# Meeso1/nmmo

Measured on AMD Instinct MI355X. Metric: agent-steps/sec (whole node), 128-agent envs at 1/2/4/8 MI355X, higher is better.
Workload: dtype int16

## Files before the change

### nmmo_amd/csrc/agent_obs.h

```cpp
#pragma once

#include <utility>

#include "kernels.h"
#include "wire.h"

namespace nmmo {

#ifndef NMMO_AO_WAVES
#define NMMO_AO_WAVES 4
#define NMMO_AO_AGENTS 16
#endif
constexpr int kAoWaves = NMMO_AO_WAVES;
constexpr int kAoAgents = NMMO_AO_AGENTS;
constexpr int kAoRows = kMaxSlots / 64;
constexpr uint32_t kAoEmpty = 0xFFFFFFFFu;
static_assert(kSize <= 256 && kMaxSlots <= 2 * 256 && kMaxSlots % 64 == 0, "packed entity word; two slots per thread (>= 256 threads)");
__host__ __device__ constexpr int ao_stride(int S) { return ((S + 1) >> 1 | 1) << 1; }
__host__ __device__ constexpr size_t ao_columns_lds(int S) {
  return ((size_t)NMMO_N_ENTITY_COLS * ao_stride(S) * 2 + 15) & ~(size_t)15;
}
constexpr size_t kAoPkBytes = (size_t)(kMaxSlots + 64) * 4;
__host__ __device__ constexpr size_t ao_entity_lds(int S) { return ao_columns_lds(S) + kAoPkBytes; }
__host__ __device__ inline uint32_t ao_pack(int slot, int row, int col, bool immune, bool danger, bool player) {
  return (uint32_t)(row & 255) | (uint32_t)(slot & 255) << 8 | (uint32_t)(col & 255) << 16 | (uint32_t)(slot >> 8) << 24 |
         (immune ? 1u << 25 : 0u) | (danger ? 1u << 26 : 0u) | (player ? 1u << 27 : 0u);
}
__device__ __forceinline__ int ao_slot(uint32_t w) { return (int)(((w >> 8) & 255u) | ((w >> 16) & 256u)); }
__device__ __forceinline__ int ao_row(uint32_t w) { return (int)(w & 255u); }
__device__ __forceinline__ int ao_col(uint32_t w) { return (int)((w >> 16) & 255u); }
__device__ __forceinline__ bool ao_immune(uint32_t w) { return (w >> 25) & 1u; }
__device__ __forceinline__ bool ao_danger(uint32_t w) { return (w >> 26) & 1u; }
__device__ __forceinline__ bool ao_player(uint32_t w) { return (w >> 27) & 1u; }
typedef unsigned short ao_u16x2 __attribute__((ext_vector_type(2)));
__device__ __forceinline__ bool ao_in_window(uint32_t w, uint32_t rc) {
  ao_u16x2 d = __builtin_bit_cast(ao_u16x2, w & 0x00FF00FFu) - __builtin_bit_cast(ao_u16x2, rc) +
               (ao_u16x2){(unsigned short)kVision, (unsigned short)kVision};
  return (d.x > d.y ? d.x : d.y) <= 2 * kVision;
}
static_assert(kMaxSlots <= 512 && kSize <= 255, "packed entity word");

__device__ __forceinline__ int ao_lane() {
  int l = (int)(threadIdx.x & 63u);
  asm volatile("" : "+v"(l));
  return l;
}

__device__ __forceinline__ uint64_t low_bits(int n) { return n >= 64 ? ~0ull : n <= 0 ? 0ull : (1ull << n) - 1ull; }
template <int L>
__device__ __forceinline__ int writelane(int v, int x) {
  static_assert(L >= 0 && L < 64, "lane");
  int sv = __builtin_amdgcn_readfirstlane(v);
  asm volatile("" : "+s"(sv));
  asm volatile("v_writelane_b32 %0, %1, %2" : "+v"(x) : "s"(sv), "n"(L));
  return x;
}
template <int kLane0, int kIdx0, int... D>
__device__ __forceinline__ int writelanes_(const uint32_t* img, int x, std::integer_sequence<int, D...>) {
  ((x = writelane<kLane0 + D>((int)img[kIdx0 + D], x)), ...);
  return x;
}
template <int kLane0, int kIdx0, int kN>
__device__ __forceinline__ int writelanes(const uint32_t* img, int x) {
  return writelanes_<kLane0, kIdx0>(img, x, std::make_integer_sequence<int, kN>{});
}

template <int kOff, int kN, int kW>
__device__ __forceinline__ void put_field(uint32_t (&img)[kW], uint64_t lo, uint64_t hi) {
  static_assert((kOff + kN + 31) / 32 <= kW, "image size");
#pragma unroll
  for (int d = kOff / 32; d <= (kOff + kN - 1) / 32; d++) {
    const int st = 32 * d - kOff;
    uint32_t x;
    if (st < 0) x = (uint32_t)(lo << (-st));
    else if (st == 0) x = (uint32_t)lo;
    else if (st < 64) x = (uint32_t)((lo >> st) | (hi << (64 - st)));
    else x = (uint32_t)(hi >> (st - 64));
    img[d] |= x;
  }
}

constexpr int kAoStageIt = (NMMO_N_ENTITY_COLS * (kMaxSlots / 8) + 255) / 256;
struct AoStage {
  uint4 x[kAoStageIt];
  int al[2], ds[2];
  int nm, mv;
};
template <bool kAligned = true>
__device__ __forceinline__ void ao_stage_load(const ObsParams& p, int e, AoStage& r) {
  const int S = p.S, tid = threadIdx.x;
  const int16_t* E = p.ent + (size_t)e * NMMO_NF * S;
  const int w4 = S / 8;
  const int nw = NMMO_N_ENTITY_COLS * w4;
  r.nm = p.mcount[e];
  r.mv = p.mlist[(size_t)e * NMMO_MARKET_ROWS + min(tid, NMMO_MARKET_ROWS - 1)];
  if constexpr (kAligned) {
#pragma unroll
    for (int k = 0; k < kAoStageIt; k++) {
      const int i = tid + (int)blockDim.x * k;
      const int f = i / w4, j = i - f * w4;
      r.x[k] = i < nw ? reinterpret_cast<const uint4*>(E + (size_t)f * S)[j] : make_uint4(0u, 0u, 0u, 0u);
    }
  }
#pragma unroll
  for (int u = 0; u < 2; u++) {
    const int s = min(tid + (int)blockDim.x * u, S - 1);
    r.al[u] = E[F_ALIVE * S + s];
    r.ds[u] = E[F_DS_ROW * S + s];
  }
}
template <bool kAligned = true>
__device__ __forceinline__ void ao_stage_store(const ObsParams& p, int e, int16_t* T, uint32_t* pk, const AoStage& r) {
  const int S = p.S, P = p.P, Sp = ao_stride(S), tid = threadIdx.x;
  const int16_t* E = p.ent + (size_t)e * NMMO_NF * S;
  const int w4 = S / 8;
  const int nw = NMMO_N_ENTITY_COLS * w4;
  constexpr int kIt = kAoStageIt;
  const int(&al)[2] = r.al;
  const int(&ds)[2] = r.ds;
  if constexpr (kAligned) {
#pragma unroll
    for (int k = 0; k < kIt; k++) {
      const int i = tid + (int)blockDim.x * k;
      if (i < nw) {
        const int f = i / w4, j = i - f * w4;
        uint32_t* d = reinterpret_cast<uint32_t*>(T + f * Sp) + 4 * j;
        d[0] = r.x[k].x;
        d[1] = r.x[k].y;
        d[2] = r.x[k].z;
        d[3] = r.x[k].w;
      }
    }
    for (int i = tid + (int)blockDim.x * kIt; i < nw; i += blockDim.x) {
      const int f = i / w4, j = i - f * w4;
      const uint4 y = reinterpret_cast<const uint4*>(E + (size_t)f * S)[j];
      uint32_t* d = reinterpret_cast<uint32_t*>(T + f * Sp) + 4 * j;
      d[0] = y.x;
      d[1] = y.y;
      d[2] = y.z;
      d[3] = y.w;
    }
  } else {
    for (int i = tid; i < NMMO_N_ENTITY_COLS * S; i += blockDim.x) {
      const int f = i / S;
      T[f * Sp + i - f * S] = E[i];
    }
  }
  for (int k = tid; k < kMaxSlots + 64; k += blockDim.x) pk[k] = kAoEmpty;
  __syncthreads();
#pragma unroll
  for (int u = 0; u < 2; u++) {
    const int s = tid + (int)blockDim.x * u;
    if (s < S && al[u] && (unsigned)(ds[u] - 1) < (unsigned)S) {
      const bool player = s < P;
      const bool immune = player && T[F_TIME_ALIVE * Sp + s] < p.spawn_immunity;
      const bool danger = T[F_NPC_TYPE * Sp + s] > 1;
      pk[ds[u] - 1] = ao_pack(s, T[F_ROW * Sp + s], T[F_COL * Sp + s], immune, danger, player);
    }
  }
  __syncthreads();
}
__device__ __forceinline__ uint2 ao_listing_load(const ObsParams& p, int e, const AoStage& r) {
  const int own = min((r.mv >> 16) & 255, p.P - 1), slot = min((r.mv >> 24) & 15, kInv - 1);
  return p.items[((size_t)e * p.P + own) * kInv + slot];
}

constexpr int kAoWinRowBytes = 20;
constexpr int kAoWinAgentBytes = 15 * kAoWinRowBytes;
__host__ __device__ constexpr size_t ao_win_lds(int agents = kAoAgents) {
  return (size_t)agents * kAoWinAgentBytes + (size_t)agents * kInv * 8;
}
__device__ __forceinline__ int ao_clamp_pos(int x) { return min(max(x, kVision), kSize - 1 - kVision); }
struct AoNoop {
  __device__ void operator()() const {}
};
template <int kAgents = kAoAgents, int kRowDw = kAoWinRowBytes / 4, typename F = AoNoop, typename B = AoNoop>
__device__ inline void ao_stage_windows(const ObsParams& p, int e, int g, const int16_t* T, int Sp, uint32_t* ws, uint2* is,
                                        F before_barrier = F(), B before_writes = B()) {
  static_assert(kRowDw == 4 || kRowDw == 5, "window row: 5 aligned dwords, or 4 realigned");
  const int tid = threadIdx.x, P = p.P;
  const int la = tid / 15, row = tid - 15 * la, a = g * kAgents + la;
  const bool win = tid < kAgents * 15 && a < P;
  uint32_t d[5] = {0u, 0u, 0u, 0u, 0u};
  if (win) {
    const int r = ao_clamp_pos(T[F_ROW * Sp + a]), c = ao_clamp_pos(T[F_COL * Sp + a]);
    const int base = (r - kVision + row) * kSize + c - kVision;
    const uint32_t* src = reinterpret_cast<const uint32_t*>(p.mat + (size_t)e * kTiles) + (base >> 2);
#pragma unroll
    for (int k = 0; k < 5; k++) d[k] = src[k];
    if constexpr (kRowDw == 4) {
#pragma unroll
      for (int k = 0; k < 4; k++) d[k] = __builtin_amdgcn_alignbyte(d[k + 1], d[k], (uint32_t)(c - kVision) & 3u);
    }
  }
  uint2 iw = make_uint2(0u, 0u);
  const bool itm = tid < kAgents * kInv && g * kAgents + tid / kInv < P;
  if (itm) iw = p.items[((size_t)e * P + g * kAgents) * kInv + tid];
  before_writes();
  if (win) {
#pragma unroll
    for (int k = 0; k < kRowDw; k++) ws[tid * kRowDw + k] = d[k];
  }
  if (tid < kAgents * kInv) is[tid] = iw;
  before_barrier();
  __syncthreads();
}
template <int kRowBytes = kAoWinRowBytes>
__device__ __forceinline__ void ao_win_offsets(int (&wo)[2]) {
  wo[0] = wo[1] = 0;
#pragma unroll
  for (int i = 0; i < 4; i++) {
    const int t = lane_id() + 64 * i;
    const int o = t < 225 ? (t / 15) * kRowBytes + t % 15 : 0;
    wo[i >> 1] |= o << (16 * (i & 1));
  }
}
__device__ __forceinline__ int ao_win_off(const int (&wo)[2], int i) { return (wo[i >> 1] >> (16 * (i & 1))) & 0xFFFF; }

__device__ __forceinline__ int ao_compact(const uint32_t (&pr)[kAoRows], int S, int r, int c, uint32_t* visw) {
  int nvis = 0;
  const uint32_t rc = (uint32_t)r | (uint32_t)c << 16;
#pragma unroll
  for (int i = 0; i < kAoRows; i++) {
    if (64 * i >= S) break;
    const uint32_t x = pr[i];
    const bool in = ao_in_window(x, rc);
    const uint64_t b = __ballot(in);
    const int pos = nvis + __popcll(b & lanes_below());
    if (in && pos < kNObs) visw[pos] = x;
    nvis += __popcll(b);
  }
  return nvis;
}

__device__ __forceinline__ void ao_window_offsets(int (&mo)[2]) {
  mo[0] = mo[1] = 0;
#pragma unroll
  for (int i = 0; i < 4; i++) {
    const int t = lane_id() + 64 * i;
    const int o = t < 225 ? (t / 15 - kVision) * kSize + t % 15 - kVision : 0;
    mo[i >> 1] |= (o & 0xFFFF) << (16 * (i & 1));
  }
}
__device__ __forceinline__ int ao_window_off(const int (&mo)[2], int i) {
  return (int)(int16_t)(uint16_t)((uint32_t)mo[i >> 1] >> (16 * (i & 1)));
}

static_assert(F_ALCHEMY_LEVEL == F_MELEE_LEVEL + 14 && F_FISHING_LEVEL == F_MELEE_LEVEL + 6 &&
                  F_HERBALISM_LEVEL == F_MELEE_LEVEL + 8, "skill level fields");
__host__ __device__ constexpr uint64_t ao_req_lut() {
  uint64_t m = 0;
  for (int t = 0; t < 16; t++) {
    const int k = (t >= T_SPEAR && t <= T_WAND) ? t - T_SPEAR : (t >= T_WHETSTONE && t <= T_RUNES) ? t - T_WHETSTONE
                  : (t >= T_ROD && t <= T_CHISEL) ? 3 + t - T_ROD : 8;
    m |= (uint64_t)k << (4 * t);
  }
  return m;
}
static_assert(T_RATION == 16 && T_POTION == 17, "requirement table: ration -> fishing, potion -> herbalism");
__device__ __forceinline__ uint64_t ao_usable_ballot(const int16_t* T, int Sp, int ti, uint2 it, bool have) {
  const int lane = ao_lane();
  int lv = 0;
  if (lane < 8) {
    lv = T[(F_MELEE_LEVEL + 2 * lane) * Sp + ti];
  } else if (lane == 8) {
    lv = max((int)T[F_MELEE_LEVEL * Sp + ti], max((int)T[F_RANGE_LEVEL * Sp + ti], (int)T[F_MAGE_LEVEL * Sp + ti]));
  }
  const int type = it_type(it);
  const int k = type < 16 ? (int)((ao_req_lut() >> (4 * type)) & 15u) : type == T_RATION ? 3 : type == T_POTION ? 4 : 8;
  const int req = __shfl(lv, k);
  const bool eq = type >= T_HAT && type <= T_RUNES && it_equipped(it);
  return __ballot(have && !it_price(it) && (eq || it_level(it) <= req));
}

struct AoSections {
  uint64_t s0, s1[2], s3, s4, s5[2], s6[2], s7[2], s8, s9, s10[2], s11;
};
struct AoAgent {
  int a, ti, r, c, gold, aid, nv, ninv, prev_price;
  uint32_t mv;
};
template <bool kWrap>
__device__ __forceinline__ AoSections ao_sections(const ObsParams& p, const int16_t* T, int Sp, const uint32_t* visw,
                                                 const AoAgent& g, uint2 it) {
  const bool combat = (p.systems & NMMO_SYS_COMBAT) != 0;
  const bool item = (p.systems & NMMO_SYS_ITEM) != 0;
  const bool exch = item && (p.systems & NMMO_SYS_EXCHANGE) != 0;
  const bool no_give = kWrap && (p.wflags & kWrapObsNoGive);
  const bool no_danger = kWrap && (p.wflags & kWrapObsNoDangerous);
  const int lane = ao_lane();
  AoSections x;
  x.s1[0] = x.s1[1] = x.s5[0] = x.s5[1] = x.s7[0] = x.s7[1] = 0ull;
#pragma unroll
  for (int h = 0; h < 2; h++) {
    if (64 * h >= g.nv) break;
    const int k = 64 * h + lane;
    bool tgt = false, st = false;
    if (k < g.nv) {
      const uint32_t w = visw[k];
      const int q = ao_slot(w);
      tgt = combat && q != g.a && linf(g.r, g.c, ao_row(w), ao_col(w)) <= 3 && !ao_immune(w) &&
            !(no_danger && ao_danger(w));
      st = ao_player(w) && q != g.a && ao_row(w) == g.r && ao_col(w) == g.c;
    }
    x.s1[h] = __ballot(tgt);
    const uint64_t sb = __ballot(st);
    if (item && !no_give) x.s5[h] = sb;
    if (exch && !no_give) x.s7[h] = sb;
  }
  x.s1[1] |= 1ull << (kNObs - 64);
  x.s5[1] |= 1ull << (kNObs - 64);
  x.s7[1] |= 1ull << (kNObs - 64);
  const bool have = lane < g.ninv;
  const bool fr = have && !it_equipped(it) && !it_price(it);
  const uint64_t bfr = __ballot(fr);
  x.s3 = (item ? bfr : 0ull) | 1ull << kInv;
  x.s4 = (item && !no_give ? bfr : 0ull) | 1ull << kInv;
  x.s9 = (exch ? __ballot(have && !it_equipped(it)) : 0ull) | 1ull << kInv;
  x.s11 = (item ? ao_usable_ballot(T, Sp, g.ti, it, have) : 0ull) | 1ull << kInv;
  x.s0 = combat ? low_bits(kSecN[0]) : 0ull;
  x.s6[0] = x.s6[1] = x.s10[0] = x.s10[1] = 0ull;
  if (exch) {
    const int ng = no_give ? min(g.gold, 1) : min(g.gold, kSecN[6]);
    x.s6[0] = low_bits(ng);
    x.s6[1] = low_bits(ng - 64);
    x.s10[0] = low_bits(kSecN[10]);
    x.s10[1] = low_bits(kSecN[10] - 64);
    if constexpr (kWrap) {
      const int pp = g.prev_price;
      if ((p.wflags & kWrapObsPrice) && pp >= 0 && pp < kSecN[10]) {
        const uint64_t clr = ~(1ull << (pp & 63));
        if (pp < 64) x.s10[0] &= clr;
        else x.s10[1] &= clr;
      }
    }
  }
  x.s8 = g.mv;
  return x;
}

template <bool kFlat, int kW>
__device__ __forceinline__ void ao_image(const AoSections& x, uint32_t (&img)[kW]) {
#pragma unroll
  for (int d = 0; d < kW; d++) img[d] = 0u;
#define AO_PUT(k, lo, hi) put_field<kFlat ? sec_flat(k) : sec_wire(k), kSecN[k], kW>(img, lo, hi)
  AO_PUT(0, x.s0, 0ull);
  AO_PUT(1, x.s1[0], x.s1[1]);
  AO_PUT(3, x.s3, 0ull);
  AO_PUT(4, x.s4, 0ull);
  AO_PUT(5, x.s5[0], x.s5[1]);
  AO_PUT(6, x.s6[0], x.s6[1]);
  AO_PUT(7, x.s7[0], x.s7[1]);
  AO_PUT(8, x.s8, 0ull);
  AO_PUT(9, x.s9, 0ull);
  AO_PUT(10, x.s10[0], x.s10[1]);
  AO_PUT(11, x.s11, 0ull);
#undef AO_PUT
}

}
```

### nmmo_amd/csrc/capi.hip

```cpp
#include <math.h>
#include <stdlib.h>
#include <string.h>

#include <algorithm>
#include <map>
#include <mutex>
#include <vector>

#include "host_api.h"
#include "kernels.h"
#include "wire.h"

using namespace nmmo;

#define HIP_TRY(expr)                                                                    \
  do {                                                                                   \
    hipError_t _e = (expr);                                                              \
    if (_e != hipSuccess) return fail(NMMO_E_HIP, "%s: %s", #expr, hipGetErrorString(_e)); \
  } while (0)

struct NmmoHandle {
  NmmoConfig cfg;
  NmmoLayout layout;
  DevState st;
  int device;
  int32_t* d_env = nullptr;
  int16_t* d_ent = nullptr;
  int16_t* d_ring = nullptr;
  uint8_t* d_mat = nullptr;
  uint32_t* d_dep = nullptr;
  int32_t* d_foreign = nullptr;
  uint8_t* d_bank = nullptr;
  float* d_task = nullptr;
  uint64_t* d_seeds = nullptr;
  uint2* d_items = nullptr;
  int16_t* d_iring = nullptr;
  int32_t* d_mlist = nullptr;
  int32_t* d_mcount = nullptr;
  int32_t* d_events = nullptr;
  NmmoTask* d_tasks = nullptr;
  int32_t* d_assign = nullptr;
  NmmoTaskState* d_tstate = nullptr;
  uint16_t* d_wcount = nullptr;
  int32_t* d_wmcount = nullptr;
  uint16_t* d_wrank = nullptr;
  uint32_t* d_wpk = nullptr;
  uint64_t* d_zrow = nullptr;
  uint64_t* d_zext = nullptr;
  bool zskip = true;
  bool wire_fuse = true;
  const void* zbuf = nullptr;
  uint64_t ztag = 0;
  unsigned long long* d_rows_out = nullptr;
  uint8_t* d_recs = nullptr;
  int32_t* d_recs_fault = nullptr;
  const void* last_native = nullptr;
  bool native_fresh = false;
  bool wrap_on = false;
  NmmoWrapperConfig wc{};
  NmmoWrapState* d_ws = nullptr;
  uint32_t* d_uniq = nullptr;
  int32_t* d_wenv = nullptr;
  uint64_t* d_task_cum = nullptr;
  unsigned long long* d_wdrop = nullptr;
  NmmoAgentInfo* d_info = nullptr;
  bool timing = false;
  int t_count = 0;
  std::vector<hipEvent_t> ev;
};
static constexpr int kTimingCap = 8192;

static float half_to_float(uint16_t h) {
  uint32_t s = (uint32_t)(h >> 15) << 31, e = (h >> 10) & 31, m = h & 1023, bits;
  if (e == 0) {
    if (m == 0) {
      bits = s;
    } else {
      int sh = 0;
      while (!(m & 1024)) { m <<= 1; sh++; }
      m &= 1023;
      bits = s | ((uint32_t)(127 - 15 - sh + 1) << 23) | (m << 13);
    }
  } else if (e == 31) {
    bits = s | 0x7F800000u | (m << 13);
  } else {
    bits = s | ((e + 112) << 23) | (m << 13);
  }
  float f;
  memcpy(&f, &bits, 4);
  return f;
}

extern "C" {

int32_t nmmo_abi_version(void) { return NMMO_ABI_VERSION; }
const char* nmmo_build_info(void) {
  return NMMO_BUILD_INFO
#ifdef NMMO_STAMPS
         " stamps=1"
#endif
      ;
}
const char* nmmo_last_error(void) { return g_err.c_str(); }

void nmmo_default_config(NmmoConfig* c) {
  memset(c, 0, sizeof(*c));
  c->abi_version = NMMO_ABI_VERSION;
  c->player_n = 128;
  c->npc_n = 256;
  c->horizon = 1024;
  c->map_n = 256;
  c->spawn_immunity = 20;
  c->early_stop_agent_num = 0;
  c->resilient_u32 = 858993459u;
  c->systems = NMMO_SYS_ALL;
  c->obs_layout = NMMO_OBS_FLAT;
  c->task_embed_dim = 2048;
  c->task_num_tick = 1024;
  c->event_cap = 4096;
  c->map_seed = 0;
  c->env_index_base = 0;
}

int nmmo_layout(const NmmoConfig* cfg, NmmoLayout* L) {
  if (!cfg || !L) return fail(NMMO_E_INVALID, "null argument");
  memset(L, 0, sizeof(*L));
  L->act_heads = NMMO_N_ACTION_HEADS;
  int* offs[NMMO_N_ACTION_HEADS] = {
      &L->off_mask_attack_style, &L->off_mask_attack_target, &L->off_mask_buy,
      &L->off_mask_destroy, &L->off_mask_give_item, &L->off_mask_give_target,
      &L->off_mask_givegold_price, &L->off_mask_givegold_target, &L->off_mask_move,
      &L->off_mask_sell_item, &L->off_mask_sell_price, &L->off_mask_use};
  for (int h = 0; h < NMMO_N_ACTION_HEADS; h++) {
    L->act_dims[h] = kSecN[h];
    *offs[h] = sec_flat(h);
  }
  L->off_agent_id = kFlatId;
  L->off_current_tick = kFlatTick;
  L->off_entity = kFlatEntity;
  L->off_inventory = kFlatInv;
  L->off_market = kFlatMarket;
  L->off_task = kFlatTask;
  L->off_tile = flat_tile(cfg->task_embed_dim);
  L->obs_elems = flat_elems(cfg->task_embed_dim);
  L->entity_rows = kNObs; L->entity_cols = NMMO_N_ENTITY_COLS;
  L->inventory_rows = kInv; L->item_cols = kItemCols; L->market_rows = NMMO_MARKET_ROWS;
  L->tile_rows = kWinTiles; L->tile_cols = kTileCols;
  const int npc = (cfg->systems & NMMO_SYS_NPC) ? cfg->npc_n : 0;
  L->slots = cfg->player_n + npc;
  L->nf = NMMO_NF;
  L->ne = NMMO_NE;
  L->state_bytes_per_env = (size_t)NMMO_NE * 4 + (size_t)NMMO_NF * L->slots * 2 +
                           (size_t)L->slots * 2 + NMMO_MAP_TILES +
                           (size_t)cfg->player_n * NMMO_INV_SLOTS * 8 +
                           (size_t)NMMO_INV_SLOTS * cfg->player_n * 2 + (size_t)cfg->player_n * 4 +
                           (size_t)cfg->player_n * sizeof(NmmoTaskState);
  return NMMO_OK;
}

int32_t nmmo_n_envs(const NmmoHandle* h) { return h ? h->st.n_envs : 0; }

void nmmo_destroy(NmmoHandle* h) {
  if (!h) return;
  (void)hipSetDevice(h->device);
  for (hipEvent_t e : h->ev) (void)hipEventDestroy(e);
  void* bufs[] = {h->d_env,  h->d_ent,   h->d_ring,  h->d_mat,   h->d_dep,   h->d_bank,
                  h->d_task, h->d_seeds, h->d_items, h->d_iring, h->d_mlist, h->d_mcount,
                  h->d_events, h->d_tasks, h->d_assign, h->d_tstate, h->d_ws, h->d_uniq, h->d_wenv, h->d_wdrop, h->d_task_cum,
                  h->d_wcount, h->d_wmcount, h->d_wrank, h->d_wpk, h->d_foreign, h->d_zrow, h->d_zext};
  for (void* b : bufs)
    if (b) (void)hipFree(b);
  delete h;
}

int nmmo_create(const NmmoConfig* cfg, int32_t n_envs, uint64_t seed, int32_t device,
                const uint16_t* task_embedding, NmmoHandle** out) {
  if (!cfg || !out) return fail(NMMO_E_INVALID, "null argument");
  *out = nullptr;
  if (cfg->abi_version != NMMO_ABI_VERSION)
    return fail(NMMO_E_INVALID, "abi_version %d != %d", cfg->abi_version, NMMO_ABI_VERSION);
  if (n_envs <= 0) return fail(NMMO_E_INVALID, "n_envs must be > 0");
  if (cfg->player_n <= 0 || cfg->player_n > 128) return fail(NMMO_E_INVALID, "player_n in 1..128");
  if (cfg->npc_n < 0 || cfg->npc_n > 256) return fail(NMMO_E_INVALID, "npc_n in 0..256");
  if (cfg->map_n <= 0) return fail(NMMO_E_INVALID, "map_n must be > 0");
  if (cfg->horizon <= 0 || cfg->task_num_tick <= 0) return fail(NMMO_E_INVALID, "horizon/task_num_tick");
  if (cfg->task_embed_dim < 0 || cfg->task_embed_dim > 65536) return fail(NMMO_E_INVALID, "task_embed_dim");
  if (cfg->event_cap < 0 || cfg->event_cap > (1 << 24)) return fail(NMMO_E_INVALID, "event_cap in 0..2^24");
  if (cfg->obs_layout != NMMO_OBS_NONE && cfg->obs_layout != NMMO_OBS_FLAT && cfg->obs_layout != NMMO_OBS_NATIVE &&
      cfg->obs_layout != NMMO_OBS_WIRE)
    return fail(NMMO_E_INVALID, "obs_layout %d", cfg->obs_layout);
  NmmoHandle* h = new NmmoHandle();
  h->cfg = *cfg;
  h->device = device;
  nmmo_layout(cfg, &h->layout);
  const int P = cfg->player_n, N = (cfg->systems & NMMO_SYS_NPC) ? cfg->npc_n : 0, S = P + N;
  auto cleanup_fail = [&](int code) { nmmo_destroy(h); return code; };
  if (hipSetDevice(device) != hipSuccess) return cleanup_fail(fail(NMMO_E_HIP, "hipSetDevice(%d)", device));
  const size_t n = (size_t)n_envs;
#define ALLOC(ptr, bytes)                                                               \
  if (hipMalloc((void**)&(ptr), (bytes)) != hipSuccess)                                  \
    return cleanup_fail(fail(NMMO_E_NOMEM, "hipMalloc %zu bytes for %s", (size_t)(bytes), #ptr)); \
  if (hipMemset((ptr), 0, (bytes)) != hipSuccess) return cleanup_fail(fail(NMMO_E_HIP, "hipMemset"));
  ALLOC(h->d_env, n * NMMO_NE * 4);
  ALLOC(h->d_ent, n * NMMO_NF * S * 2);
  ALLOC(h->d_ring, n * S * 2);
  ALLOC(h->d_mat, n * NMMO_MAP_TILES);
  ALLOC(h->d_dep, n * kBitmapWords * 4);
  ALLOC(h->d_foreign, 8);
  ALLOC(h->d_bank, (size_t)cfg->map_n * NMMO_MAP_TILES);
  ALLOC(h->d_task, (size_t)(cfg->task_embed_dim > 0 ? cfg->task_embed_dim : 1) * 4);
  ALLOC(h->d_seeds, n * 8);
  ALLOC(h->d_items, n * P * NMMO_INV_SLOTS * 8);
  ALLOC(h->d_iring, n * NMMO_INV_SLOTS * P * 2);
  ALLOC(h->d_mlist, n * NMMO_MARKET_ROWS * 4);
  ALLOC(h->d_mcount, n * 4);
  if (cfg->event_cap > 0) ALLOC(h->d_events, n * (size_t)cfg->event_cap * NMMO_EVENT_COLS * 4);
  ALLOC(h->d_tasks, sizeof(NmmoTask));
  ALLOC(h->d_assign, n * P * 4);
  ALLOC(h->d_tstate, n * P * sizeof(NmmoTaskState));
  if (cfg->obs_layout == NMMO_OBS_NATIVE) {
    ALLOC(h->d_wcount, n * P * 2);
    ALLOC(h->d_wmcount, n * 4);
  }
  if (cfg->obs_layout == NMMO_OBS_FLAT || cfg->obs_layout == NMMO_OBS_NATIVE) {
    ALLOC(h->d_zrow, n * P * 16);
  }
  if (cfg->obs_layout == NMMO_OBS_FLAT) {
    ALLOC(h->d_zext, n * P * kZext * 8);
  }
  {
    const char* rz = getenv("NMMO_OBS_REZERO");
    h->zskip = !(rz && rz[0] == '1');
    const char* wf = getenv("NMMO_WIRE_FUSE");
    h->wire_fuse = !(wf && wf[0] == '0');
  }
  if (cfg->obs_layout == NMMO_OBS_WIRE) {
    ALLOC(h->d_wrank, n * (size_t)kMaxSlots * 2);
    ALLOC(h->d_wpk, n * (size_t)kMaxSlots * 4);
  }
#undef ALLOC
  if (init_kernels() != hipSuccess) return cleanup_fail(fail(NMMO_E_HIP, "kernel attributes"));
  if (task_embedding && cfg->task_embed_dim > 0) {
    std::vector<float> t(cfg->task_embed_dim);
    for (int k = 0; k < cfg->task_embed_dim; k++) t[k] = half_to_float(task_embedding[k]);
    if (hipMemcpy(h->d_task, t.data(), t.size() * 4, hipMemcpyHostToDevice) != hipSuccess)
      return cleanup_fail(fail(NMMO_E_HIP, "task upload"));
  }
  h->st = DevState{h->d_env,   h->d_ent,   h->d_ring,  h->d_mat,    h->d_dep, h->d_bank,
                   h->d_items, h->d_iring, h->d_mlist, h->d_mcount, h->d_events,
                   h->d_tasks, h->d_assign, nullptr, h->d_tstate, 1,            0,           0, 0, n_envs, P,
                   N,          S,          seed,       nullptr,     *cfg,      h->d_foreign,
                   h->d_foreign + 1, nullptr, 0};
  {
    NmmoTask t;
    memset(&t, 0, sizeof(t));
    t.term[0].pred = PRED_TICK_GE;
    t.term[0].a = cfg->task_num_tick;
    if (hipMemcpy(h->d_tasks, &t, sizeof(t), hipMemcpyHostToDevice) != hipSuccess)
      return cleanup_fail(fail(NMMO_E_HIP, "task table upload"));
  }
  if (launch_mapgen(cfg->map_seed, cfg->map_n, h->d_bank, nullptr) != hipSuccess ||
      hipDeviceSynchronize() != hipSuccess)
    return cleanup_fail(fail(NMMO_E_HIP, "map generation failed: %s", hipGetErrorString(hipGetLastError())));
  *out = h;
  return NMMO_OK;
}

static ObsParams obs_params(NmmoHandle* h, void* obs) {
  ObsParams p;
  const bool native = h->cfg.obs_layout == NMMO_OBS_NATIVE, wire = h->cfg.obs_layout == NMMO_OBS_WIRE;
  p.env = h->d_env; p.ent = h->d_ent; p.mat = h->d_mat; p.task = h->d_task;
  p.obs = native || wire ? nullptr : (float*)obs;
  p.nat = native ? (uint8_t*)obs : nullptr;
  p.wire = wire ? (uint8_t*)obs : nullptr;
  p.items = h->d_items; p.mlist = h->d_mlist; p.mcount = h->d_mcount; p.assign = h->d_assign;
  p.n_envs = h->st.n_envs; p.P = h->st.P; p.S = h->st.S;
  p.task_dim = h->cfg.task_embed_dim; p.systems = h->cfg.systems;
  p.spawn_immunity = h->cfg.spawn_immunity;
  p.row_map = nullptr;
  p.env_list = nullptr;
  p.n_list = 0;
  p.wcount = native ? h->d_wcount : nullptr;
  p.wmcount = native ? h->d_wmcount : nullptr;
  p.wrank = wire ? h->d_wrank : nullptr;
  p.wpk = wire ? h->d_wpk : nullptr;
  p.fault = h->d_foreign + 1;
  p.zrow = h->d_zrow;
  p.zst = h->d_zrow ? h->d_zrow + (size_t)h->st.n_envs * h->st.P : nullptr;
  p.zext = h->d_zext;
  p.ztag = h->d_zrow && h->zskip && obs && obs == h->zbuf ? h->ztag : 0;
  p.rows_out = h->d_rows_out;
  p.counted = 0;
  p.recs = nullptr;
  p.fault_dst = nullptr;
  p.rew = nullptr;
  p.term = p.trunc = p.mask = nullptr;
  p.ws = h->wrap_on ? h->d_ws : nullptr;
  p.wflags = 0;
  if (h->wrap_on) {
    if (h->wc.kind == NMMO_WRAP_START_KIT) p.wflags |= kWrapObsPrice;
    if (h->wc.disable_give) p.wflags |= kWrapObsNoGive;
    if (h->wc.donot_attack_dangerous_npc) p.wflags |= kWrapObsNoDangerous;
  }
  return p;
}

static WrapParams wrap_params(NmmoHandle* h, const int32_t* actions, float* rew, const uint8_t* term,
                              const uint8_t* trunc, const uint8_t* mask) {
  WrapParams p;
  p.env = h->d_env; p.ent = h->d_ent; p.items = h->d_items; p.events = h->d_events;
  p.tstate = h->d_tstate; p.actions = actions; p.rew = rew; p.term = term; p.trunc = trunc;
  p.mask = mask; p.ws = h->d_ws; p.uniq = h->d_uniq; p.wenv = h->d_wenv; p.wdrop = h->d_wdrop; p.info = h->d_info;
  p.wc = h->wc; p.n_envs = h->st.n_envs; p.P = h->st.P; p.S = h->st.S; p.evcap = h->cfg.event_cap;
  p.items_on = (h->cfg.systems & NMMO_SYS_ITEM) != 0;
  p.env_list = nullptr;
  p.n_list = 0;
  return p;
}

int nmmo_reset(NmmoHandle* h, const uint64_t* env_seeds, void* obs, uint8_t* mask, void* stream) {
  if (!h) return fail(NMMO_E_INVALID, "null handle");
  hipStream_t s = (hipStream_t)stream;
  HIP_TRY(hipSetDevice(h->device));
  if (env_seeds) {
    HIP_TRY(hipMemcpyAsync(h->d_seeds, env_seeds, (size_t)h->st.n_envs * 8, hipMemcpyHostToDevice, s));
    HIP_TRY(hipStreamSynchronize(s));
  }
  HIP_TRY(launch_tick(h->st, nullptr, env_seeds ? h->d_seeds : nullptr, nullptr, nullptr, nullptr,
                      mask, 1, s));
  HIP_TRY(hipMemsetAsync(h->d_foreign, 0, 4, s));
  if (h->wrap_on) HIP_TRY(launch_wrap(wrap_params(h, nullptr, nullptr, nullptr, nullptr, nullptr), 0, s));
  const bool do_obs = obs && h->cfg.obs_layout != NMMO_OBS_NONE;
  if (do_obs) HIP_TRY(launch_obs(obs_params(h, obs), s));
  if (do_obs) h->last_native = obs;
  h->native_fresh = do_obs;
  return NMMO_OK;
}

__global__ void end_episodes_kernel(int32_t* env, const uint8_t* m, int n) {
  const int e = blockIdx.x * blockDim.x + threadIdx.x;
  if (e < n && m[e]) env[(size_t)e * NMMO_NE + E_DONE] = 1;
}

int nmmo_end_episodes(NmmoHandle* h, const uint8_t* dev_env_mask, void* stream) {
  if (!h || !dev_env_mask) return fail(NMMO_E_INVALID, "null argument");
  const int n = h->st.n_envs;
  HIP_TRY(hipSetDevice(h->device));
  hipLaunchKernelGGL(end_episodes_kernel, dim3((n + 255) / 256), dim3(256), 0, (hipStream_t)stream, h->d_env,
                     dev_env_mask, n);
  HIP_TRY(hipGetLastError());
  return NMMO_OK;
}

static int step_impl(NmmoHandle* h, const int32_t* env_ids, int32_t n_ids, const int32_t* actions, void* obs,
                     float* rew, uint8_t* term, uint8_t* trunc, uint8_t* mask, void* stream) {
  if (!h) return fail(NMMO_E_INVALID, "null handle");
  if (!actions || !rew || !term || !trunc || !mask)
    return fail(NMMO_E_INVALID, "actions/rew/term/trunc/mask must be device pointers");
  HIP_TRY(hipSetDevice(h->device));
  hipStream_t s = (hipStream_t)stream;
  const bool rec = h->timing && h->t_count < kTimingCap;
  hipEvent_t* ev = rec ? &h->ev[(size_t)h->t_count * 4] : nullptr;
  DevState st = h->st;
  st.env_list = env_ids;
  st.n_list = n_ids;
  const bool do_obs = obs && h->cfg.obs_layout != NMMO_OBS_NONE;
  if (do_obs && h->cfg.obs_layout == NMMO_OBS_WIRE && !env_ids && !h->wrap_on && h->wire_fuse &&
      st.cfg.systems == NMMO_SYS_ALL && st.S == 384 && st.P == 128) {
    st.wf.wire = (uint8_t*)obs;
    st.wf.wrank = h->d_wrank;
    st.wf.wpk = h->d_wpk;
    st.wf.n_envs = st.n_envs;
    st.wf.spawn_immunity = h->cfg.spawn_immunity;
  }
  if (rec) HIP_TRY(hipEventRecord(ev[0], s));
  HIP_TRY(launch_tick(st, actions, nullptr, rew, term, trunc, mask, 0, s));
  if (rec) HIP_TRY(hipEventRecord(ev[1], s));
  if (h->wrap_on) {
    WrapParams wp = wrap_params(h, actions, rew, term, trunc, mask);
    wp.env_list = env_ids;
    wp.n_list = n_ids;
    HIP_TRY(launch_wrap(wp, 0, s));
  }
  if (rec) HIP_TRY(hipEventRecord(ev[2], s));
  if (do_obs) {
    ObsParams op = obs_params(h, obs);
    op.env_list = env_ids;
    op.n_list = n_ids;
    op.counted = st.wf.wire != nullptr;
    if (op.wire && h->d_recs) {
      op.recs = h->d_recs;
      op.fault_dst = h->d_recs_fault;
      op.rew = rew;
      op.term = term;
      op.trunc = trunc;
      op.mask = mask;
    }
    HIP_TRY(launch_obs(op, s));
  }
  if (do_obs) h->last_native = obs;
  h->native_fresh = do_obs && !env_ids;
  if (rec) {
    HIP_TRY(hipEventRecord(ev[3], s));
    h->t_count++;
  }
  return NMMO_OK;
}

int nmmo_step(NmmoHandle* h, const int32_t* actions, void* obs, float* rew, uint8_t* term,
              uint8_t* trunc, uint8_t* mask, void* stream) {
  return step_impl(h, nullptr, 0, actions, obs, rew, term, trunc, mask, stream);
}

int nmmo_step_envs(NmmoHandle* h, const int32_t* env_ids, int32_t n_ids, const int32_t* actions, void* obs,
                   float* rew, uint8_t* term, uint8_t* trunc, uint8_t* mask, void* stream) {
  if (!h || !env_ids) return fail(NMMO_E_INVALID, "null handle / env_ids");
  if (n_ids < 0 || n_ids > h->st.n_envs) return fail(NMMO_E_INVALID, "n_ids %d not in 0..%d", n_ids, h->st.n_envs);
  if (h->cfg.obs_layout == NMMO_OBS_WIRE && obs)
    return fail(NMMO_E_INVALID, "nmmo_step_envs: the wire layout packs every env of the handle (use nmmo_step)");
  return step_impl(h, env_ids, n_ids, actions, obs, rew, term, trunc, mask, stream);
}

__global__ void fault_into_kernel(const int32_t* word, int32_t* dst) {
  const int32_t w = *word;
  if (w) atomicCAS(dst, 0, w);
}

int nmmo_fault_into(NmmoHandle* h, int32_t* dev_dst, void* stream) {
  if (!h || !dev_dst) return fail(NMMO_E_INVALID, "null argument");
  HIP_TRY(hipSetDevice(h->device));
  hipLaunchKernelGGL(fault_into_kernel, dim3(1), dim3(1), 0, (hipStream_t)stream, h->d_foreign + 1, dev_dst);
  HIP_TRY(hipGetLastError());
  return NMMO_OK;
}

int nmmo_inject_fault(NmmoHandle* h, int32_t fault) {
  if (!h) return fail(NMMO_E_INVALID, "null handle");
  HIP_TRY(hipSetDevice(h->device));
  HIP_TRY(hipDeviceSynchronize());
  HIP_TRY(hipMemcpy(h->d_foreign + 1, &fault, 4, hipMemcpyHostToDevice));
  return NMMO_OK;
}

int nmmo_observe(NmmoHandle* h, void* obs, void* stream) {
  if (!h || !obs) return fail(NMMO_E_INVALID, "null argument");
  if (h->cfg.obs_layout == NMMO_OBS_NONE) return fail(NMMO_E_INVALID, "handle built with NMMO_OBS_NONE");
  HIP_TRY(hipSetDevice(h->device));
  HIP_TRY(launch_obs(obs_params(h, obs), (hipStream_t)stream));
  h->last_native = obs;
  h->native_fresh = true;
  return NMMO_OK;
}

int nmmo_expand_obs(NmmoHandle* h, const void* native, float* flat, int32_t n_envs, void* stream) {
  if (!h || !native || !flat) return fail(NMMO_E_INVALID, "null argument");
  if (n_envs <= 0) return fail(NMMO_E_INVALID, "n_envs must be > 0");
  ObsParams p = obs_params(h, nullptr);
  p.nat = (uint8_t*)native;
  p.obs = flat;
  p.n_envs = n_envs;
  HIP_TRY(launch_expand(p, (hipStream_t)stream));
  return NMMO_OK;
}

namespace {
struct VmmAlloc {
  size_t bytes;
  std::vector<hipMemGenericAllocationHandle_t> chunks;
};
std::mutex g_vmm_mu;
std::map<void*, VmmAlloc> g_vmm;
constexpr size_t kVmmChunk = (size_t)64 << 20;
}

int nmmo_dev_alloc(int32_t device, uint64_t bytes, void** out) {
  if (!out || bytes == 0) return fail(NMMO_E_INVALID, "null out / zero bytes");
  *out = nullptr;
  HIP_TRY(hipSetDevice(device));
  int vmm = 0;
  HIP_TRY(hipDeviceGetAttribute(&vmm, hipDeviceAttributeVirtualMemoryManagementSupported, device));
  if (!vmm) return fail(NMMO_E_INVALID, "device %d has no virtual memory management (hipMemCreate / hipMemMap)", device);
  hipMemAllocationProp prop = {};
  prop.type = hipMemAllocationTypePinned;
  prop.location.type = hipMemLocationTypeDevice;
  prop.location.id = device;
  size_t gran = 0;
  HIP_TRY(hipMemGetAllocationGranularity(&gran, &prop, hipMemAllocationGranularityMinimum));
  const size_t chunk = gran > kVmmChunk ? gran : (kVmmChunk / gran) * gran;
  const size_t total = (bytes + chunk - 1) / chunk * chunk;
  void* va = nullptr;
  HIP_TRY(hipMemAddressReserve(&va, total, chunk, nullptr, 0));
  VmmAlloc a{total, {}};
  size_t mapped = 0;
  auto undo = [&]() {
    for (size_t i = 0; i < mapped; i++) (void)hipMemUnmap((char*)va + i * chunk, chunk);
    for (auto c : a.chunks) (void)hipMemRelease(c);
    (void)hipMemAddressFree(va, total);
  };
  for (size_t off = 0; off < total; off += chunk) {
    hipMemGenericAllocationHandle_t hdl;
    if (hipMemCreate(&hdl, chunk, &prop, 0) != hipSuccess) {
      undo();
      return fail(NMMO_E_NOMEM, "hipMemCreate of a %zu-byte chunk (%zu of %zu mapped)", chunk, off, total);
    }
    a.chunks.push_back(hdl);
    if (hipMemMap((char*)va + off, chunk, 0, hdl, 0) != hipSuccess) {
      undo();
      return fail(NMMO_E_HIP, "hipMemMap at offset %zu", off);
    }
    mapped++;
  }
  hipMemAccessDesc acc = {};
  acc.location = prop.location;
  acc.flags = hipMemAccessFlagsProtReadWrite;
  if (hipMemSetAccess(va, total, &acc, 1) != hipSuccess) {
    undo();
    return fail(NMMO_E_HIP, "hipMemSetAccess");
  }
  std::lock_guard<std::mutex> lk(g_vmm_mu);
  g_vmm[va] = std::move(a);
  *out = va;
  return NMMO_OK;
}

int nmmo_dev_free(void* ptr) {
  if (!ptr) return NMMO_OK;
  VmmAlloc a;
  {
    std::lock_guard<std::mutex> lk(g_vmm_mu);
    auto it = g_vmm.find(ptr);
    if (it == g_vmm.end()) return fail(NMMO_E_INVALID, "pointer was not returned by nmmo_dev_alloc");
    a = std::move(it->second);
    g_vmm.erase(it);
  }
  HIP_TRY(hipDeviceSynchronize());
  const size_t chunk = a.chunks.empty() ? a.bytes : a.bytes / a.chunks.size();
  for (size_t i = 0; i < a.chunks.size(); i++) HIP_TRY(hipMemUnmap((char*)ptr + i * chunk, chunk));
  for (auto c : a.chunks) HIP_TRY(hipMemRelease(c));
  const char* fr = getenv("NMMO_DEVMEM_FREE_VA");
  if (fr && fr[0] == '1') HIP_TRY(hipMemAddressFree(ptr, a.bytes));
  return NMMO_OK;
}

int nmmo_set_step_records(NmmoHandle* h, uint8_t* dev_records, int32_t* dev_fault) {
  if (!h) return fail(NMMO_E_INVALID, "null handle");
  if (dev_records && h->cfg.obs_layout != NMMO_OBS_WIRE)
    return fail(NMMO_E_INVALID, "nmmo_set_step_records: step records come with the wire obs layout");
  if (dev_fault && !dev_records) return fail(NMMO_E_INVALID, "nmmo_set_step_records: dev_fault without records");
  h->d_recs = dev_records;
  h->d_recs_fault = dev_fault;
  return NMMO_OK;
}

int nmmo_obs_bind(NmmoHandle* h, const void* obs) {
  if (!h) return fail(NMMO_E_INVALID, "null handle");
  if (!h->d_zrow) return obs ? fail(NMMO_E_INVALID, "nmmo_obs_bind: flat or native obs layouts only") : NMMO_OK;
  HIP_TRY(hipSetDevice(h->device));
  HIP_TRY(hipDeviceSynchronize());
  HIP_TRY(hipMemset(h->d_zrow, 0, (size_t)h->st.n_envs * h->st.P * 8));
  h->zbuf = obs;
  h->ztag = obs ? h->ztag + 1 : h->ztag;
  return NMMO_OK;
}

int nmmo_obs_invalidate(NmmoHandle* h, void* stream) {
  if (!h) return fail(NMMO_E_INVALID, "null handle");
  if (!h->d_zrow) return NMMO_OK;
  HIP_TRY(hipSetDevice(h->device));
  HIP_TRY(hipMemsetAsync(h->d_zrow, 0, (size_t)h->st.n_envs * h->st.P * 8, (hipStream_t)stream));
  return NMMO_OK;
}

__global__ void obs_forget_envs_kernel(uint64_t* zrow, const int32_t* ids, int n_ids, int n_envs, int P) {
  const int i = blockIdx.x, e = ids[i];
  if ((unsigned)e >= (unsigned)n_envs) return;
  for (int a = threadIdx.x; a < P; a += blockDim.x) zrow[(size_t)e * P + a] = 0;
}

int nmmo_obs_invalidate_envs(NmmoHandle* h, const int32_t* env_ids, int32_t n_ids, void* stream) {
  if (!h) return fail(NMMO_E_INVALID, "null handle");
  if (n_ids < 0 || n_ids > h->st.n_envs) return fail(NMMO_E_INVALID, "n_ids %d not in 0..%d", n_ids, h->st.n_envs);
  if (n_ids > 0 && !env_ids) return fail(NMMO_E_INVALID, "null env_ids");
  if (!h->d_zrow || n_ids == 0) return NMMO_OK;
  HIP_TRY(hipSetDevice(h->device));
  hipLaunchKernelGGL(obs_forget_envs_kernel, dim3(n_ids), dim3(128), 0, (hipStream_t)stream, h->d_zrow, env_ids,
                     n_ids, h->st.n_envs, h->st.P);
  HIP_TRY(hipGetLastError());
  return NMMO_OK;
}

__global__ void obs_forget_tile_kernel(uint64_t* zst, const int32_t* ids, int n_envs, int P) {
  const int e = ids ? ids[blockIdx.x] : (int)blockIdx.x;
  if ((unsigned)e >= (unsigned)n_envs) return;
  for (int a = threadIdx.x; a < P; a += blockDim.x) zst[(size_t)e * P + a] |= kZsTile;
}

int nmmo_obs_invalidate_sections(NmmoHandle* h, const int32_t* env_ids, int32_t n_ids, uint32_t sections,
                                 void* stream) {
  if (!h) return fail(NMMO_E_INVALID, "null handle");
  if (!env_ids) n_ids = h->st.n_envs;
  if (n_ids < 0 || n_ids > h->st.n_envs) return fail(NMMO_E_INVALID, "n_ids %d not in 0..%d", n_ids, h->st.n_envs);
  if (!h->d_zrow || n_ids == 0 || sections == 0) return NMMO_OK;
  HIP_TRY(hipSetDevice(h->device));
  const bool tile_only = sections == NMMO_OBS_SEC_TILE && h->cfg.obs_layout == NMMO_OBS_FLAT;
  if (!tile_only) {
    if (!env_ids) {
      HIP_TRY(hipMemsetAsync(h->d_zrow, 0, (size_t)h->st.n_envs * h->st.P * 8, (hipStream_t)stream));
      return NMMO_OK;
    }
    return nmmo_obs_invalidate_envs(h, env_ids, n_ids, stream);
  }
  hipLaunchKernelGGL(obs_forget_tile_kernel, dim3(n_ids), dim3(128), 0, (hipStream_t)stream,
                     h->d_zrow + (size_t)h->st.n_envs * h->st.P, env_ids, h->st.n_envs, h->st.P);
  HIP_TRY(hipGetLastError());
  return NMMO_OK;
}

int nmmo_set_obs_counter(NmmoHandle* h, uint64_t* dev_rows) {
  if (!h) return fail(NMMO_E_INVALID, "null handle");
  if (dev_rows) {
    HIP_TRY(hipSetDevice(h->device));
    hipPointerAttribute_t at;
    if (hipPointerGetAttributes(&at, dev_rows) != hipSuccess || at.type != hipMemoryTypeDevice ||
        at.device != h->device) {
      (void)hipGetLastError();
      return fail(NMMO_E_INVALID, "nmmo_set_obs_counter: not device memory of device %d", h->device);
    }
  }
  h->d_rows_out = reinterpret_cast<unsigned long long*>(dev_rows);
  return NMMO_OK;
}

int64_t nmmo_wire_header_bytes(int32_t n_envs, int32_t player_n) {
  if (n_envs <= 0 || player_n <= 0 || player_n > 128) return fail(NMMO_E_INVALID, "n_envs > 0, player_n in 1..128");
  return wire_header_bytes(n_envs, player_n);
}

int64_t nmmo_wire_max_bytes(int32_t n_envs, int32_t player_n) {
  const int64_t hdr = nmmo_wire_header_bytes(n_envs, player_n);
  if (hdr < 0) return hdr;
  const int64_t rec = wire_record_bytes(wire_count_word(kNObs, kInv));
  return hdr + (int64_t)n_envs * (wire_table_bytes(kMaxSlots) + (int64_t)player_n * rec + NMMO_NATIVE_MARKET_BYTES);
}

int nmmo_wire_pack(NmmoHandle* h, const void* native, void* wire, void* stream) {
  if (!h || !native || !wire) return fail(NMMO_E_INVALID, "null argument");
  if (h->cfg.obs_layout != NMMO_OBS_NATIVE || !h->d_wcount)
    return fail(NMMO_E_INVALID, "nmmo_wire_pack needs a handle created with NMMO_OBS_NATIVE");
  if (native != h->last_native)
    return fail(NMMO_E_INVALID, "nmmo_wire_pack: `native` is not the buffer the handle's last obs gather wrote");
  if (!h->native_fresh)
    return fail(NMMO_E_INVALID, "nmmo_wire_pack: a tick ran after the last obs gather without one (stale native obs)");
  HIP_TRY(hipSetDevice(h->device));
  const int exch = (h->cfg.systems & NMMO_SYS_ITEM) && (h->cfg.systems & NMMO_SYS_EXCHANGE);
  HIP_TRY(launch_wire_pack(h->d_wcount, h->d_wmcount, (const uint8_t*)native, (uint8_t*)wire, h->st.n_envs, h->st.P,
                           h->d_ent, h->st.S, exch, (hipStream_t)stream));
  return NMMO_OK;
}

int nmmo_wire_check(const void* wire, int32_t n_envs, int32_t player_n, const int64_t* dev_expect_total,
                    int32_t* dev_status, void* stream) {
  if (!wire || !dev_status) return fail(NMMO_E_INVALID, "null argument");
  if (n_envs <= 0 || player_n <= 0 || player_n > 128) return fail(NMMO_E_INVALID, "n_envs > 0, player_n in 1..128");
  HIP_TRY(launch_wire_check((const uint8_t*)wire, n_envs, player_n, dev_expect_total, dev_status, (hipStream_t)stream));
  return NMMO_OK;
}

int nmmo_wire_check_many(const void* const* wires, const int32_t* n_envs, const int64_t* const* dev_expect_totals,
                         int32_t n_bufs, int32_t player_n, int32_t* dev_status, void* stream) {
  if (!wires || !n_envs || !dev_status) return fail(NMMO_E_INVALID, "null argument");
  if (n_bufs < 1 || n_bufs > kMaxCheckBufs) return fail(NMMO_E_INVALID, "n_bufs %d not in 1..%d", n_bufs, kMaxCheckBufs);
  if (player_n <= 0 || player_n > 128) return fail(NMMO_E_INVALID, "player_n in 1..128");
  WireCheckBatch b;
  memset(&b, 0, sizeof(b));
  b.count = n_bufs;
  for (int i = 0; i < n_bufs; i++) {
    if (!wires[i] || n_envs[i] <= 0) return fail(NMMO_E_INVALID, "buffer %d: null wire / n_envs <= 0", i);
    b.wire[i] = (const uint8_t*)wires[i];
    b.n[i] = n_envs[i];
    b.expect[i] = dev_expect_totals ? dev_expect_totals[i] : nullptr;
  }
  HIP_TRY(launch_wire_check_many(b, player_n, dev_status, (hipStream_t)stream));
  return NMMO_OK;
}

struct SizesRowArgs {
  const int64_t* w[kMaxCheckBufs];
  int n;
};
__global__ void sizes_row_kernel(SizesRowArgs a, int32_t* fault, int64_t* row) {
  const int j = threadIdx.x;
  if (j < a.n) row[j] = *a.w[j];
// ... 566 lines not shown
```

### nmmo_amd/csrc/flat_obs.hip

```cpp
#include "agent_obs.h"

namespace nmmo {

#ifndef NMMO_FO_ABL
#define NMMO_FO_ABL 0
#endif
#ifndef NMMO_FO_STAMPS
#define NMMO_FO_STAMPS 0
#endif
#if NMMO_FO_STAMPS
constexpr int kFoStamps = 12;
__device__ uint64_t fo_stamp_buf[1 << 17][kFoStamps];
__device__ uint64_t fo_wave_buf[1 << 15][6];
#define FO_STAMP(k) fst[k] = __builtin_amdgcn_s_memtime()
#else
#define FO_STAMP(k) (void)0
#endif
#ifndef NMMO_FO_XCD
#define NMMO_FO_XCD 1
#endif
#ifndef NMMO_FO_TILE_SKIP
#define NMMO_FO_TILE_SKIP 0
#endif
#ifndef NMMO_FO_TASK_BATCH
#define NMMO_FO_TASK_BATCH 8
#endif
constexpr int kFoTaskBatch = NMMO_FO_TASK_BATCH;
constexpr int kFoStagedListings = 64;
constexpr int kFoChunks = 25;
static_assert(kFoChunks * 64 >= kMaskN + 2 && (kFoChunks - 1) * 64 < kMaskN, "mask chunks");
static_assert(kFlatId == kMaskN && kFlatTick == kMaskN + 1 && kFlatEntity == kMaskN + 2, "id, tick in the last chunk");
static_assert(kWireBuyLo / 64 == 1 && (kWireBuyLo + NMMO_MARKET_ROWS) / 64 == 17, "Buy.MarketItem: chunks 1 to 17");

constexpr int kFoVisw = (kNObs + 3) & ~3;
constexpr int kFoWinRowBytes = 16, kFoWinAgentBytes = 15 * kFoWinRowBytes;
constexpr size_t kFoWinBytes = (size_t)kAoAgents * kFoWinAgentBytes, kFoItemBytes = (size_t)kAoAgents * kInv * 8;
static_assert(F_COL == F_ROW + 1 && kAoPkBytes <= kFoWinBytes, "shared LDS regions");
__host__ __device__ constexpr bool fo_items_in_T(int S) {
  return (size_t)2 * ao_stride(S) * 2 >= kFoItemBytes && (F_ROW * ao_stride(S) * 2) % 8 == 0;
}
constexpr int kFoListPool = NMMO_MARKET_ROWS * 2 + kFoStagedListings * 8;
__host__ __device__ constexpr int fo_staged(int nm) {
  return nm < ((kFoListPool - ((2 * nm + 7) & ~7)) >> 3) ? nm : (kFoListPool - ((2 * nm + 7) & ~7)) >> 3;
}
static_assert(fo_staged(NMMO_MARKET_ROWS) == kFoStagedListings && fo_staged(256) == 256 && fo_staged(257) == 255 &&
                  fo_staged(0) == 0 && kFoListPool % 16 == 0, "listings' pool");
__host__ __device__ constexpr size_t fo_lds_bytes(int S) {
  return ao_columns_lds(S) + (size_t)kFoListPool +
         (size_t)kAoWaves * kFoVisw * 4 + kFoWinBytes + (fo_items_in_T(S) ? 0 : kFoItemBytes);
}
constexpr size_t kFoLdsGranule = 1280;
static_assert(kAoAgents != 16 ||
                  (5 * fo_lds_bytes(kMaxSlots) <= 160 * 1024 && fo_items_in_T(kMaxSlots) &&
                   5 * ((fo_lds_bytes(kMaxSlots) + kFoLdsGranule - 1) / kFoLdsGranule * kFoLdsGranule) <= 160 * 1024),
              "5 workgroups per CU");

template <int kSh>
__device__ __forceinline__ uint64_t fo_shift(uint64_t lo, uint64_t hi) {
  if constexpr (kSh >= 64) {
    return 0ull;
  } else if constexpr (kSh > 0) {
    return lo << kSh;
  } else if constexpr (kSh == 0) {
    return lo;
  } else if constexpr (-kSh < 64) {
    return (lo >> (-kSh)) | (hi << (64 + kSh));
  } else if constexpr (-kSh < 128) {
    return hi >> (-kSh - 64);
  } else {
    return 0ull;
  }
}
template <int kK, int kC>
__device__ __forceinline__ uint64_t fo_sec(uint64_t lo, uint64_t hi) {
  constexpr int off = sec_flat(kK), n = kSecN[kK];
  if constexpr (off >= 64 * kC + 64 || off + n <= 64 * kC) return 0ull;
  else return fo_shift<off - 64 * kC>(lo, hi);
}
template <int kC>
__device__ __forceinline__ uint64_t fo_chunk(const AoSections& x) {
  return fo_sec<0, kC>(x.s0, 0ull) | fo_sec<1, kC>(x.s1[0], x.s1[1]) | fo_sec<3, kC>(x.s3, 0ull) |
         fo_sec<4, kC>(x.s4, 0ull) | fo_sec<5, kC>(x.s5[0], x.s5[1]) | fo_sec<6, kC>(x.s6[0], x.s6[1]) |
         fo_sec<7, kC>(x.s7[0], x.s7[1]) | fo_sec<8, kC>(x.s8, 0ull) | fo_sec<9, kC>(x.s9, 0ull) |
         fo_sec<10, kC>(x.s10[0], x.s10[1]) | fo_sec<11, kC>(x.s11, 0ull);
}
__device__ __forceinline__ float fo_bit(uint64_t m) { return __builtin_amdgcn_inverse_ballot_w64(m) ? 1.f : 0.f; }
__device__ __forceinline__ void fo_st(float* row, uint32_t idx, float v) {
  *reinterpret_cast<float*>(reinterpret_cast<char*>(row) + (idx << 2)) = v;
}

constexpr int kFoTail0 = (kWireBuyLo + NMMO_MARKET_ROWS) / 64;
__host__ __device__ constexpr int fo_slot(int c) { return c < 2 ? c : c - kFoTail0 + 2; }
static_assert(fo_slot(kFoChunks - 1) == 9 && kZext == 10 + 1 + 12, "tracked chunks | position | items");
struct FoImg {
  bool ext;
  uint32_t lo, hi;
  int j10;
  int nimg;
  int nst;
};
__device__ __forceinline__ uint64_t fo_prev(const FoImg& g, int slot) {
  return (uint64_t)(uint32_t)__builtin_amdgcn_readlane((int)g.lo, g.j10 + slot) |
         (uint64_t)(uint32_t)__builtin_amdgcn_readlane((int)g.hi, g.j10 + slot) << 32;
}
template <int kC>
__device__ __forceinline__ void fo_put(float* row, FoImg& g, uint64_t m, float aid, float tick) {
  constexpr int sl = fo_slot(kC);
  const int lane = ao_lane();
  const bool same = g.ext && m == fo_prev(g, sl);
  if constexpr (kC == kFoChunks - 1) {
    constexpr int n = kMaskN - 64 * kC;
    if (!same) {
      if (lane < n + 2) fo_st(row, 64 * kC + lane, lane < n ? fo_bit(m) : lane == n ? aid : tick);
      g.nst += n + 2;
    } else {
      if (lane == n + 1) fo_st(row, 64 * kC + lane, tick);
      g.nst += 1;
    }
  } else if (!same) {
    fo_st(row, 64 * kC + lane, fo_bit(m));
    g.nst += 64;
  }
  g.nimg = writelane<2 * sl>((int)(uint32_t)m, g.nimg);
  g.nimg = writelane<2 * sl + 1>((int)(uint32_t)(m >> 32), g.nimg);
}
template <int kC>
__device__ __forceinline__ void fo_tail_chunks(float* row, FoImg& g, const AoSections& x, uint64_t buy17, float aid,
                                               float tick) {
  if constexpr (kC < kFoChunks) {
    uint64_t m = fo_chunk<kC>(x);
    if constexpr (kC == kFoTail0) m |= buy17 | 1ull << ((kWireBuyLo + NMMO_MARKET_ROWS) & 63);
    fo_put<kC>(row, g, m, aid, tick);
    fo_tail_chunks<kC + 1>(row, g, x, buy17, aid, tick);
  }
}

struct IcDesc {
  uint32_t tmA, tmB;
  uint32_t f;
};
__device__ __forceinline__ IcDesc ic_desc(int col) {
  auto bits = [](int lo, int hi) { return ((2u << hi) - 1u) & ~((1u << lo) - 1u); };
  IcDesc d{0u, 0u, 0u};
  auto bf = [&](int sel, int sh, int wd) { d.f = (uint32_t)(sel | sh << 1 | wd << 6); };
  switch (col) {
    case 0: bf(1, 16, 16); break;
    case 1: bf(0, 0, 5); break;
    case 2: d.f = 1u << 11; break;
    case 3: bf(0, 5, 4); break;
    case 5: bf(1, 0, 16); break;
    case 6: case 7: case 8:
      d.tmA = 1u << (T_SPEAR + col - 6) | 1u << (T_WHETSTONE + col - 6);
      d.f = 5u << 12 | 5u << 20;
      break;
    case 9: case 10: case 11:
      d.tmA = bits(T_HAT, T_BOTTOM);
      d.tmB = bits(T_ROD, T_CHISEL);
      d.f = 3u << 12 | 2u << 16;
      break;
    case 12: d.tmA = 1u << T_POTION; d.f = 5u << 12 | 50u << 20; break;
    case 13: d.tmA = 1u << T_RATION; d.f = 5u << 12 | 50u << 20; break;
    case 14: bf(0, 9, 1); break;
    case 15: bf(0, 10, 7); break;
    default: break;
  }
  return d;
}
__device__ __forceinline__ float ic_value(uint2 w, int owner, const IcDesc& d) {
  const int type = (int)(w.x & 31u), lvl = (int)((w.x >> 5) & 15u);
  const uint32_t bfv = __builtin_amdgcn_ubfe((d.f & 1u) ? w.y : w.x, (d.f >> 1) & 31u, (d.f >> 6) & 31u);
  const int ta = (int)((d.tmA >> type) & 1u), tb = (int)((d.tmB >> type) & 1u);
  const int mult = ta * (int)((d.f >> 12) & 15u) + tb * (int)((d.f >> 16) & 15u);
  return (float)((int)bfv + (int)((d.f >> 11) & 1u) * owner + mult * lvl + ((ta | tb) ? (int)(d.f >> 20) : 0));
}
static_assert(T_POTION < 32 && T_RATION < 32 && T_WHETSTONE + 2 < 32, "item type masks");

__device__ __forceinline__ int fo_compact(const uint32_t (&pr)[kAoRows], int r, int c, uint32_t* visw) {
  int nvis = 0;
  const uint32_t rc = (uint32_t)r | (uint32_t)c << 16;
#pragma unroll
  for (int i = 0; i < kAoRows; i++) {
    const bool in = ao_in_window(pr[i], rc);
    const uint64_t b = __ballot(in);
    const int pos = nvis + __popcll(b & lanes_below());
    if (in && pos < kNObs) visw[pos] = pr[i];
    nvis += __popcll(b);
  }
  return nvis;
}

typedef const __attribute__((address_space(4))) ObsParams* FoArgs;

template <bool kWrap, int kS, bool kAligned = true>
__global__ void __launch_bounds__(64 * kAoWaves) __attribute__((amdgpu_waves_per_eu(5, 5))) flat_obs_kernel(ObsParams p) {
  extern __shared__ __attribute__((aligned(16))) unsigned char smem[];
  const int S = kS ? kS : p.S, P = p.P, Sp = ao_stride(S), tdim = p.task_dim, elems = kFlatTask + tdim + kTileN;
  int16_t* T = reinterpret_cast<int16_t*>(smem);
  uint16_t* mpo = reinterpret_cast<uint16_t*>(smem + ao_columns_lds(S));
  uint32_t* visw_all = reinterpret_cast<uint32_t*>(mpo) + kFoListPool / 4;
  uint2* mtop = reinterpret_cast<uint2*>(visw_all) - 1;
  uint32_t* wst = visw_all + kAoWaves * kFoVisw;
  uint32_t* pk = wst;
  uint2* ist = reinterpret_cast<uint2*>(fo_items_in_T(S) ? smem + (size_t)F_ROW * Sp * 2
                                                         : reinterpret_cast<unsigned char*>(wst) + kFoWinBytes);
#if NMMO_FO_XCD
  int el, g;
  ao_env_group(p.env_list ? p.n_list : p.n_envs, (p.P + kAoAgents - 1) / kAoAgents, el, g);
#else
  const int el = blockIdx.x, g = blockIdx.y;
#endif
  const int e = p.env_list ? p.env_list[el] : el, tid = threadIdx.x, lane = lane_id();
  if ((unsigned)e >= (unsigned)p.n_envs) return;
  if (NMMO_FO_ABL & 128) return;
#if NMMO_FO_STAMPS
  uint64_t wst_[6];
  wst_[0] = __builtin_amdgcn_s_memtime();
#endif
  const int w = __builtin_amdgcn_readfirstlane(wave_id());
  AoStage sg;
  ao_stage_load<kAligned>(p, e, sg);
  const int16_t* E = p.ent + (size_t)e * NMMO_NF * S;
  constexpr int kPerWave = kAoAgents / kAoWaves;
  const int abase = g * kAoAgents + w;
  int my_task = 0, my_prev = -1, my_alive = 0;
  uint64_t my_z = 0, my_s = 0;
  const bool mine = lane < kPerWave && abase + kAoWaves * lane < P;
  {
    const int aj = min(abase + kAoWaves * min(lane, kPerWave - 1), P - 1);
    const size_t ai = (size_t)e * P + aj;
    my_task = p.assign[ai];
    my_alive = E[F_ALIVE * S + aj];
    if (p.zrow) {
      my_z = p.zrow[ai];
      my_s = p.zst[ai];
    }
    if constexpr (kWrap)
      if (p.ws) my_prev = p.ws[ai].prev_price;
  }
  ao_stage_store<kAligned>(p, e, T, pk, sg);
  if (!mine) {
    my_task = 0, my_prev = -1, my_alive = 0;
    my_z = my_s = 0;
  }
  uint32_t my_rc;
  {
    const int aj = min(abase + kAoWaves * min(lane, kPerWave - 1), P - 1);
    my_rc = (uint32_t)(uint16_t)T[F_ROW * Sp + aj] | (uint32_t)(uint16_t)T[F_COL * Sp + aj] << 16;
  }
#if NMMO_FO_STAMPS
  wst_[1] = __builtin_amdgcn_s_memtime();
#endif

  uint32_t pr[kAoRows];
#pragma unroll
  for (int i = 0; i < kAoRows; i++) pr[i] = pk[lane + 64 * i];
  uint32_t* visw = visw_all + w * kFoVisw;
  const uint8_t* wsb = reinterpret_cast<const uint8_t*>(wst);
  const float tickf = (float)p.env[(size_t)e * NMMO_NE + E_TICK];
  const bool exch = (p.systems & NMMO_SYS_ITEM) && (p.systems & NMMO_SYS_EXCHANGE);

  const bool zvl = p.ztag && my_z == p.ztag;
  const bool zzl = zvl && (my_s & kZsZero);
  const uint64_t zvalid = __ballot(zvl), zzero = __ballot(zzl), ztask = __ballot(zvl && !zzl && zs_task(my_s) == my_task);
  const uint64_t zextv = __ballot(zvl && !zzl && (my_s & kZsExt));
  const uint64_t ztile = __ballot(zvl && (my_s & kZsTile));
  uint2 img = make_uint2(0u, 0u), pinv = make_uint2(0u, 0u);
  const int ja = lane < 40 ? lane / 10 : lane - 40, ji = lane / 12;
  const bool img_ok = lane < 44 && abase + kAoWaves * ja < P && ((zextv >> ja) & 1);
  const bool pinv_ok = lane < 48 && abase + kAoWaves * ji < P && ((zextv >> ji) & 1);
  if (p.zext) {
    const int aa = min(abase + kAoWaves * min(ja, kPerWave - 1), P - 1);
    const int ai = min(abase + kAoWaves * min(ji, kPerWave - 1), P - 1);
    img = reinterpret_cast<const uint2*>(p.zext)[((size_t)e * P + aa) * kZext + (lane < 40 ? lane % 10 : 10)];
    pinv = reinterpret_cast<const uint2*>(p.zext)[((size_t)e * P + ai) * kZext + 11 + min(lane, 47) % 12];
  }
  const int nm = min(max(sg.nm, 0), NMMO_MARKET_ROWS), nst = fo_staged(nm);
  const uint2 lwd = ao_listing_load(p, e, sg);
  ao_stage_windows<kAoAgents, kFoWinRowBytes / 4>(p, e, g, T, Sp, wst, ist, [&]() {
    if (tid < nm) {
      mpo[tid] = (uint16_t)(it_price(lwd) | ((sg.mv >> 16) & 255) << 8);
      if (tid < nst) mtop[-tid] = lwd;
    }
    for (int j = tid + (int)blockDim.x; j < nm; j += blockDim.x) {
      const int v = p.mlist[(size_t)e * NMMO_MARKET_ROWS + j];
      const int own = (v >> 16) & 255, slot = (v >> 24) & 15;
      const uint2 wd = p.items[((size_t)e * P + own) * kInv + slot];
      mpo[j] = (uint16_t)(it_price(wd) | own << 8);
      if (j < nst) mtop[-j] = wd;
    }
  }, []() { __syncthreads(); });
#if NMMO_FO_STAMPS
  wst_[2] = __builtin_amdgcn_s_memtime();
#endif
  asm volatile("" : "+v"(img.x), "+v"(img.y), "+v"(pinv.x), "+v"(pinv.y), "+v"(my_prev));
  if (!img_ok) img = make_uint2(0u, 0u);
  if (!pinv_ok) pinv = make_uint2(0u, 0u);
  const int my_h = !zvl ? (kNObs | NMMO_MARKET_ROWS << 12) : zzl ? 0 : (zs_hv(my_s) | zs_hm(my_s) << 12);
  int nrows = 0;
  unsigned long long nbytes = 0;
  int wo[2];
  ao_win_offsets<kFoWinRowBytes>(wo);
  int toff[4];
#pragma unroll
  for (int i = 0; i < 4; i++) {
    const int t = lane + 64 * i;
    toff[i] = ((t / 15 - kVision) & 255) | (t % 15 - kVision) * 256;
  }
  const int ef = lane & 31, eh = lane >> 5;
  const int iq = lane >> 4;
  const IcDesc icd = ic_desc(lane & 15);

#if NMMO_FO_STAMPS
  wst_[3] = __builtin_amdgcn_s_memtime();
#endif
#pragma unroll 1
  for (int j = 0; j < ((NMMO_FO_ABL & 64) ? 0 : kPerWave); j++) {
    const int a = abase + kAoWaves * j;
    if (a >= P) break;
    const int lane = ao_lane();
    FoArgs kp = (FoArgs)__builtin_amdgcn_kernarg_segment_ptr();
    asm volatile("" : "+s"(kp));
    auto grow = (__attribute__((address_space(1))) float*)(p.obs + ((NMMO_FO_ABL & 256)
        ? (size_t)(((e * P + a) & 15) + 16 * (blockIdx.x & 7)) : (size_t)e * P + a) * elems);
    asm volatile("" : "+s"(grow));
    float* row = (float*)grow;
    const bool zv = (zvalid >> j) & 1;
    const int hj = __builtin_amdgcn_readlane(my_h, j);
    const int hv = hj & 4095, hm = hj >> 12;
    if (!__builtin_amdgcn_readlane(my_alive, j)) {
      if ((zzero >> j) & 1) {
        if ((ztile >> j) & 1) {
          wave_zero(row, kFlatTask + tdim, elems);
          nbytes += 4ull * (elems - kFlatTask - tdim);
          if (lane == 0) kp->zst[(size_t)e * P + a] = kZsZero;
          nrows++;
        }
        continue;
      }
      if (zv) {
        wave_zero(row, 0, kFlatEntity + hv * NMMO_N_ENTITY_COLS);
        wave_zero(row, kFlatInv, kFlatMarket + hm * 16);
        wave_zero(row, kFlatTask, elems);
        nbytes += 4ull * (kFlatEntity + hv * NMMO_N_ENTITY_COLS + kFlatMarket + hm * 16 - kFlatInv + elems - kFlatTask);
      } else {
        wave_zero(row, 0, elems);
        nbytes += 4ull * elems;
      }
      if (lane == 0) {
        kp->zrow[(size_t)e * P + a] = kp->ztag;
        kp->zst[(size_t)e * P + a] = kZsZero;
      }
      nrows++;
      continue;
    }
    nrows++;
#if NMMO_FO_STAMPS
    uint64_t fst[kFoStamps];
#endif
    FO_STAMP(0);
    const int la = a - g * kAoAgents;
    const int rcj = __builtin_amdgcn_readlane((int)my_rc, j);
    const int r = (int16_t)(rcj & 0xFFFF), c = rcj >> 16;
    const int gold = __builtin_amdgcn_readfirstlane(T[F_GOLD * Sp + a]);
    const int aid = __builtin_amdgcn_readfirstlane(T[F_ID * Sp + a]);
    const uint8_t* wa = wsb + la * kFoWinAgentBytes;
    uint32_t wm[4];
#pragma unroll
    for (int i = 0; i < 4; i++) wm[i] = lane + 64 * i < 225 ? wa[ao_win_off(wo, i)] : 0u;
    const uint2 it = lane < kInv ? ist[la * kInv + lane] : make_uint2(0u, 0u);
    const uint32_t mv = ao_move_bits(wm[1]);
    const int ninv = __builtin_ctzll(~__ballot(lane < kInv && it_type(it) != 0));
    const int nv = (NMMO_FO_ABL & 32) ? 0 : min(fo_compact(pr, r, c, visw), kNObs);
    __builtin_amdgcn_fence(__ATOMIC_RELEASE, "wavefront");
    __builtin_amdgcn_wave_barrier();
    __builtin_amdgcn_fence(__ATOMIC_ACQUIRE, "wavefront");

    FO_STAMP(1);
    const bool ext = (zextv >> j) & 1;
    FoImg fg{ext, img.x, img.y, 10 * j, 0, 0};
    if (!(NMMO_FO_ABL & 1)) {
      AoAgent ag;
      ag.a = a;
      ag.ti = a;
      ag.r = r;
      ag.c = c;
      ag.gold = gold;
      ag.aid = aid;
      ag.nv = nv;
      ag.ninv = ninv;
      ag.prev_price = kWrap ? __builtin_amdgcn_readlane(my_prev, j) : -1;
      ag.mv = mv;
      const AoSections x = ao_sections<kWrap>(p, T, Sp, visw, ag, it);
      FO_STAMP(2);
      fg.ext = ext;
      fo_put<0>(row, fg, fo_chunk<0>(x), 0.f, 0.f);
      auto buy_word = [&](int m) {
        const int k = 64 * m + lane;
        bool bv = false;
        if (exch && k < nm) {
          const uint32_t po = mpo[k];
          bv = (int)(po & 255u) <= gold && (int)(po >> 8) != a;
        }
        return __ballot(bv);
      };
      const int nbuy = max(nm, hm);
      const int clast = max(1, min((kWireBuyLo + nbuy - 1) >> 6, 16));
      uint64_t bprev = nm > 0 ? buy_word(0) : 0ull;
      fo_put<1>(row, fg, fo_chunk<1>(x) | bprev << (kWireBuyLo & 63), 0.f, 0.f);
      FO_STAMP(3);
#pragma unroll 1
      for (int cc = 2; cc <= clast; cc++) {
        const uint64_t bcur = 64 * (cc - 1) < nm ? buy_word(cc - 1) : 0ull;
        fo_st(row, 64 * cc + lane, fo_bit(bcur << (kWireBuyLo & 63) | bprev >> (64 - (kWireBuyLo & 63))));
        bprev = bcur;
      }
      FO_STAMP(4);
      const uint64_t buy17 = nm > 15 * 64 ? bprev >> (64 - (kWireBuyLo & 63)) : 0ull;
      fo_tail_chunks<kFoTail0>(row, fg, x, buy17, (float)aid, tickf);
      nbytes += 4ull * (fg.nst + 64 * (clast - 1));
    }
    FO_STAMP(5);
    const int nv2 = (nv + 1) & ~1;
    if (!(NMMO_FO_ABL & 2)) {
      const uint32_t de = kFlatEntity + (lane - eh);
      const bool epos = (lane & 31) == F_ROW || (lane & 31) == F_COL;
      const uint32_t esh = (lane & 31) == F_COL ? 16u : 0u;
#pragma unroll 1
      for (int k0 = 0; k0 < nv2; k0 += 2) {
        const int k = k0 + eh;
        if (ef < NMMO_N_ENTITY_COLS) {
          float v = 0.f;
          if (k < nv) {
            const uint32_t vw = visw[k];
            const int tv = T[ef * Sp + ao_slot(vw)];
            v = (float)(epos ? (int)((vw >> esh) & 255u) : tv);
          }
          fo_st(row, de + k0 * NMMO_N_ENTITY_COLS, v);
        }
      }
      const int hz = max(nv2, hv);
      wave_zero(row, kFlatEntity + nv2 * NMMO_N_ENTITY_COLS, kFlatEntity + hz * NMMO_N_ENTITY_COLS);
      nbytes += 4ull * (hz * NMMO_N_ENTITY_COLS + max(nm, hm) * 16);
    }
    FO_STAMP(6);
    const int jl = (12 * j + lane) & 63;
    const uint32_t px = (uint32_t)__shfl((int)pinv.x, jl), py = (uint32_t)__shfl((int)pinv.y, jl);
    const bool inv_same = ext && __ballot(lane < kInv && (px != it.x || py != it.y)) == 0ull;
    if (!inv_same) {
#pragma unroll
      for (int h = 0; h < ((NMMO_FO_ABL & 4) ? 0 : kInv * 16 / 64); h++) {
        const int q = 4 * h + iq;
        float v = 0.f;
        if (4 * h < ninv && q < ninv) v = ic_value(ist[la * kInv + q], aid, icd);
        fo_st(row, kFlatInv + 64 * h + lane, v);
      }
      nbytes += 4ull * kInv * 16;
    }
    FO_STAMP(7);
    const int nms = (NMMO_FO_ABL & 8) ? 0 : fo_staged(nm);
    for (int k = lane; k < nms * 16; k += 64) fo_st(row, kFlatMarket + k, ic_value(mtop[-(k >> 4)], (mpo[k >> 4] >> 8) + 1, icd));
    if (nm > nms && !(NMMO_FO_ABL & 8)) {
      for (int k = nms * 16 + lane; k < nm * 16; k += 64) {
        const int q = k >> 4;
        const int v = kp->mlist[(size_t)e * NMMO_MARKET_ROWS + q];
        const uint2 wd = kp->items[((size_t)e * P + ((v >> 16) & 255)) * kInv + ((v >> 24) & 15)];
        fo_st(row, kFlatMarket + k, ic_value(wd, (mpo[q] >> 8) + 1, icd));
      }
    }
    wave_zero(row, kFlatMarket + nm * 16, kFlatMarket + max(nm, hm) * 16);
    FO_STAMP(8);
    const int task = __builtin_amdgcn_readlane(my_task, j);
    if (!((ztask >> j) & 1)) {
      const float* temb = kp->task + (size_t)task * tdim;
      int k0 = 0;
      for (; k0 + kFoTaskBatch * 64 <= tdim; k0 += kFoTaskBatch * 64) {
        float t[kFoTaskBatch];
#pragma unroll
        for (int i = 0; i < kFoTaskBatch; i++) t[i] = temb[k0 + 64 * i + lane];
#pragma unroll
        for (int i = 0; i < kFoTaskBatch; i++) fo_st(row, kFlatTask + k0 + 64 * i + lane, t[i]);
      }
      for (int k = k0 + lane; k < tdim; k += 64) fo_st(row, kFlatTask + k, temb[k]);
      nbytes += 4ull * tdim;
    }
    FO_STAMP(9);
    const uint32_t ppos = (uint32_t)__builtin_amdgcn_readlane((int)img.x, 40 + j);
    const bool tkn = NMMO_FO_TILE_SKIP && ext && !((ztile >> j) & 1);
    const bool same_r = tkn && (int)(ppos & 255u) == r, same_c = tkn && (int)((ppos >> 8) & 255u) == c;
    if (!(NMMO_FO_ABL & 16)) {
      float* dt = row + kFlatTask + tdim + 3 * lane;
#pragma unroll
      for (int i = 0; i < 4; i++) {
        if (lane + 64 * i < 225) {
          const float vr = (float)(r + ((toff[i] << 24) >> 24)), vc = (float)(c + (toff[i] >> 8)), vm = (float)wm[i];
          if (NMMO_FO_TILE_SKIP) {
            if (!same_r) dt[192 * i] = vr;
            if (!same_c) dt[192 * i + 1] = vc;
            dt[192 * i + 2] = vm;
          } else {
            typedef float f3 __attribute__((ext_vector_type(3)));
            const f3 v = {vr, vc, vm};
            __builtin_memcpy(dt + 192 * i, &v, 12);
          }
        }
      }
      nbytes += 4ull * 225 * (1 + !same_r + !same_c);
    }
    FO_STAMP(10);
    {
      uint32_t* zx = reinterpret_cast<uint32_t*>(kp->zext + ((size_t)e * P + a) * kZext);
      int wv = fg.nimg;
      if (lane == 20) wv = r | c << 8;
      if (lane == 21) wv = 0;
      if (lane < 22) zx[lane] = (uint32_t)wv;
      if (!inv_same && lane < kInv) reinterpret_cast<uint2*>(zx + 22)[lane] = it;
      if (lane == 0) {
        if (!zv) kp->zrow[(size_t)e * P + a] = kp->ztag;
        kp->zst[(size_t)e * P + a] = zs_pack(nv2, nm, task) | kZsExt;
      }
    }
#if NMMO_FO_STAMPS
    FO_STAMP(11);
    if (lane == 0 && (size_t)e * P + a < (1u << 17))
      for (int k = 0; k < kFoStamps; k++) fo_stamp_buf[(size_t)e * P + a][k] = fst[k];
#endif
    __builtin_amdgcn_fence(__ATOMIC_RELEASE, "wavefront");
    __builtin_amdgcn_wave_barrier();
    __builtin_amdgcn_fence(__ATOMIC_ACQUIRE, "wavefront");
  }
#if NMMO_FO_STAMPS
  wst_[4] = __builtin_amdgcn_s_memtime();
  wst_[5] = (uint64_t)e | (uint64_t)nrows << 32;
  {
    const size_t wi = ((size_t)blockIdx.y * gridDim.x + blockIdx.x) * kAoWaves + w;
    if (lane == 0 && wi < (1u << 15))
      for (int k = 0; k < 6; k++) fo_wave_buf[wi][k] = wst_[k];
  }
#endif
  if (p.rows_out && lane == 0 && nrows) {
    atomicAdd(&p.rows_out[2 * e], (unsigned long long)nrows);
    atomicAdd(&p.rows_out[2 * e + 1], nbytes);
  }
}

hipError_t launch_flat_obs(const ObsParams& p, hipStream_t stream) {
  if (!(p.obs && p.ztag && p.zrow)) return hipErrorInvalidValue;
  const int ne = list_grid(p.env_list, p.n_list, p.n_envs);
  if (ne <= 0) return hipSuccess;
#if NMMO_FO_XCD
  const dim3 grid(ne * ((p.P + kAoAgents - 1) / kAoAgents)), block(64 * kAoWaves);
#else
  const dim3 grid(ne, (p.P + kAoAgents - 1) / kAoAgents), block(64 * kAoWaves);
#endif
  const size_t lds = fo_lds_bytes(p.S);
  if (p.S == kMaxSlots) {
    if (p.wflags) hipLaunchKernelGGL((flat_obs_kernel<true, kMaxSlots>), grid, block, lds, stream, p);
    else hipLaunchKernelGGL((flat_obs_kernel<false, kMaxSlots>), grid, block, lds, stream, p);
  } else if (p.S % 8 != 0) {
    if (p.wflags) hipLaunchKernelGGL((flat_obs_kernel<true, 0, false>), grid, block, lds, stream, p);
    else hipLaunchKernelGGL((flat_obs_kernel<false, 0, false>), grid, block, lds, stream, p);
  } else {
    if (p.wflags) hipLaunchKernelGGL((flat_obs_kernel<true, 0>), grid, block, lds, stream, p);
    else hipLaunchKernelGGL((flat_obs_kernel<false, 0>), grid, block, lds, stream, p);
  }
  return hipGetLastError();
}

}

#if NMMO_FO_STAMPS
extern "C" __attribute__((visibility("default"))) int nmmo_debug_fo_stamps(void* host, size_t bytes) {
  if (bytes > sizeof(nmmo::fo_stamp_buf)) bytes = sizeof(nmmo::fo_stamp_buf);
  if (hipDeviceSynchronize() != hipSuccess) return -1;
  if (hipMemcpyFromSymbol(host, HIP_SYMBOL(nmmo::fo_stamp_buf), bytes) != hipSuccess) return -1;
  void* d = nullptr;
  if (hipGetSymbolAddress(&d, HIP_SYMBOL(nmmo::fo_stamp_buf)) != hipSuccess) return -1;
  return hipMemset(d, 0, sizeof(nmmo::fo_stamp_buf)) == hipSuccess && hipDeviceSynchronize() == hipSuccess ? 0 : -1;
}
extern "C" __attribute__((visibility("default"))) int nmmo_debug_fo_wave_stamps(void* host, size_t bytes) {
  if (bytes > sizeof(nmmo::fo_wave_buf)) bytes = sizeof(nmmo::fo_wave_buf);
  if (hipDeviceSynchronize() != hipSuccess) return -1;
  if (hipMemcpyFromSymbol(host, HIP_SYMBOL(nmmo::fo_wave_buf), bytes) != hipSuccess) return -1;
  void* d = nullptr;
  if (hipGetSymbolAddress(&d, HIP_SYMBOL(nmmo::fo_wave_buf)) != hipSuccess) return -1;
  return hipMemset(d, 0, sizeof(nmmo::fo_wave_buf)) == hipSuccess && hipDeviceSynchronize() == hipSuccess ? 0 : -1;
}
#endif
```

### nmmo_amd/csrc/kernels.h

```cpp
#pragma once

#include "common.h"
#include "obs_layout.h"

namespace nmmo {

constexpr int kSlimNF = 30;
__host__ __device__ constexpr bool slim_systems(uint32_t sy) {
  return (sy & (NMMO_SYS_ITEM | NMMO_SYS_EQUIPMENT | NMMO_SYS_PROFESSION | NMMO_SYS_EXCHANGE)) == 0;
}
__host__ __device__ constexpr bool slim_staged(int f) {
  return f != F_ITEM_LEVEL && f != F_MESSAGE && f != F_GOLD && !(f >= F_FISHING_LEVEL && f <= F_ALCHEMY_EXP) &&
         f != F_EQUIP_OFFENSE && f != F_EQUIP_DEFENSE;
}
__host__ __device__ constexpr int slim_const(int f, bool player) {
  return player && f >= F_FISHING_LEVEL && f <= F_ALCHEMY_EXP && ((f - F_FISHING_LEVEL) & 1) == 0 ? 1 : 0;
}

struct DevState {
  int32_t* env;
  int16_t* ent;
  int16_t* ring;
  uint8_t* mat;
  uint32_t* dep;
  const uint8_t* bank;
  uint2* items;
  int16_t* iring;
  int32_t* mlist;
  int* mcount;
  int32_t* events;
  const NmmoTask* tasks;
  int32_t* assign;
  const uint64_t* task_cum;
  NmmoTaskState* tstate;
  int n_tasks, tev;
  int tmap;
  int tsee;
  int n_envs, P, N, S;
  uint64_t seed;
  unsigned long long* counters;
  NmmoConfig cfg;
  int32_t* foreign;
  int32_t* fault;
  const int32_t* env_list;
  int n_list;
  struct WireFuse {
    uint8_t* wire;
    uint16_t* wrank;
    uint32_t* wpk;
    int n_envs;
    int spawn_immunity;
  } wf;
};
__host__ __device__ inline int list_grid(const int32_t* list, int n_list, int n) { return list ? n_list : n; }

struct ObsParams {
  const int32_t* env;
  const int16_t* ent;
  const uint8_t* mat;
  const uint2* items;
  const int32_t* mlist;
  const int* mcount;
  const float* task;
  const int32_t* assign;
  float* obs;
  uint8_t* nat;
  uint8_t* wire;
  const int* row_map;
  int n_envs, P, S, counted, task_dim;
  uint32_t systems;
  int spawn_immunity;
  const NmmoWrapState* ws;
  int wflags;
  uint16_t* wcount;
  int* wmcount;
  uint16_t* wrank;
  const int32_t* env_list;
  int n_list;
  uint32_t* wpk;
  int32_t* fault;
  uint64_t* zrow;
  uint64_t* zst;
  uint64_t ztag;
  uint64_t* zext;
  uint8_t* recs;
  int32_t* fault_dst;
  const float* rew;
  const uint8_t* term;
  const uint8_t* trunc;
  const uint8_t* mask;
  unsigned long long* rows_out;
};
constexpr uint64_t kZsZero = 1ull << 20;
constexpr uint64_t kZsExt = 1ull << 21;
constexpr uint64_t kZsTile = 1ull << 22;
constexpr int kZext = 10 + 1 + 12;
__host__ __device__ inline int zs_hv(uint64_t s) { return (int)(s & 255u); }
__host__ __device__ inline int zs_hm(uint64_t s) { return (int)((s >> 8) & 4095u); }
__host__ __device__ inline int zs_task(uint64_t s) { return (int)(uint32_t)(s >> 32); }
__host__ __device__ inline uint64_t zs_pack(int hv, int hm, int task) {
  return (uint64_t)hv | (uint64_t)hm << 8 | (uint64_t)(uint32_t)task << 32;
}
__device__ __forceinline__ uint64_t readlane_u64(uint64_t v, int j) {
  return (uint64_t)(uint32_t)__builtin_amdgcn_readlane((int)(uint32_t)v, j) |
         (uint64_t)(uint32_t)__builtin_amdgcn_readlane((int)(uint32_t)(v >> 32), j) << 32;
}
constexpr int kWrapObsPrice = 1, kWrapObsNoGive = 2, kWrapObsNoDangerous = 4;

__device__ __forceinline__ void ao_env_group(int n_envs, int G, int& e, int& g) {
  const int id = blockIdx.x;
  if ((n_envs & 7) == 0) {
    const int x = id & 7, q = id >> 3;
    g = q % G;
    e = (q / G) * 8 + x;
  } else {
    e = id / G;
    g = id - e * G;
  }
}
__device__ __forceinline__ uint32_t ao_move_bits(uint32_t wm1) {
  uint32_t b = 0u;
#pragma unroll
  for (int d = 0; d < 5; d++) {
    const int t = (kVision + dir_dr(d)) * 15 + kVision + dir_dc(d);
    if (!impassable((int)__builtin_amdgcn_readlane((int)wm1, t - 64))) b |= 1u << d;
  }
  return b;
}

struct WrapParams {
  const int32_t* env;
  const int16_t* ent;
  const uint2* items;
  const int32_t* events;
  const NmmoTaskState* tstate;
  const int32_t* actions;
  float* rew;
  const uint8_t* term;
  const uint8_t* trunc;
  const uint8_t* mask;
  NmmoWrapState* ws;
  uint32_t* uniq;
  int32_t* wenv;
  unsigned long long* wdrop;
  NmmoAgentInfo* info;
  NmmoWrapperConfig wc;
  int n_envs, P, S, evcap, items_on;
  const int32_t* env_list;
  int n_list;
};

struct PolicyParams {
  const int32_t* env;
  const int16_t* ent;
  const uint8_t* mat;
  const uint2* items;
  const int32_t* mlist;
  const int* mcount;
  int32_t* actions;
  int n_envs, P, S;
  uint32_t systems;
  int spawn_immunity;
  uint64_t seed;
};

hipError_t init_kernels();
hipError_t launch_mapgen(uint64_t seed, int map_n, uint8_t* bank, hipStream_t stream);
hipError_t launch_tick(const DevState& st, const int32_t* actions, const uint64_t* env_seeds,
                       float* rew, uint8_t* term, uint8_t* trunc, uint8_t* mask, int mode,
                       hipStream_t stream);
hipError_t launch_rebuild_dep(const DevState& st, hipStream_t stream);
hipError_t launch_obs(const ObsParams& p, hipStream_t stream);
hipError_t launch_expand(const ObsParams& p, hipStream_t stream);
hipError_t launch_wire_pack(const uint16_t* counts, const int* mcount, const uint8_t* native, uint8_t* wire, int n,
                            int P, const int16_t* ent, int S, int exch, hipStream_t s);
hipError_t launch_wire_unpack(const uint8_t* wire, uint8_t* native, int n, int P, hipStream_t s);
hipError_t launch_wire_header(const ObsParams& p, hipStream_t s);
hipError_t launch_wire_obs(const ObsParams& p, hipStream_t s);
hipError_t launch_flat_obs(const ObsParams& p, hipStream_t s);
hipError_t launch_native_obs(const ObsParams& p, hipStream_t s);
hipError_t launch_wire_check(const uint8_t* wire, int n, int P, const int64_t* expect_total, int* status,
                             hipStream_t s);
constexpr int kMaxCheckBufs = 16;
struct WireCheckBatch {
  const uint8_t* wire[kMaxCheckBufs];
  const int64_t* expect[kMaxCheckBufs];
  int n[kMaxCheckBufs];
  int count;
};
hipError_t launch_wire_check_many(const WireCheckBatch& b, int P, int* status, hipStream_t s);
hipError_t launch_wire_expand(const ObsParams& p, hipStream_t s);
hipError_t launch_store(const NmmoExperience& x, const NmmoStoreInput& in, const ObsParams* native,
                        int* scratch, hipStream_t stream);
hipError_t launch_store_records(const NmmoExperience& x, const NmmoRecordStore& rs, const NmmoStoreInput& in,
                                int P, int64_t wire_cap, int* scratch, hipStream_t stream);
constexpr int kMaxStoreInputs = 16;
struct StoreBatch {
  NmmoStoreInput in[kMaxStoreInputs];
  int64_t wire_cap[kMaxStoreInputs];
  int n, P;
  int stride;
};
struct StoreCheck {
  const int64_t* expect[kMaxStoreInputs];
  int* status;
  int* ctl;
  uint32_t mask;
};
int p2p_load(const char* path, char* err, size_t n);
int p2p_unique_id(void* id, char* err, size_t n);
int p2p_init(const void* id, int world, int rank, void** comm, char* err, size_t n);
int p2p_group(void* comm, const NmmoP2POp* ops, int n_ops, hipStream_t stream, char* err, size_t n);
int p2p_destroy(void* comm);
int store_many_scratch_ints(int n_inputs, int max_rows);
hipError_t launch_store_records_many(const NmmoExperience& x, const NmmoRecordStore& rs, const StoreBatch& b,
                                     int* scratch, hipStream_t stream, const StoreCheck* chk = nullptr);
hipError_t launch_record_gather(const ObsParams& p, const NmmoRecordStore& rs, const int32_t* idx, int n,
                                float* out, hipStream_t stream);
int store_blocks(int n_rows);
hipError_t launch_sort(const NmmoExperience& x, int32_t* idxs, int* scratch, hipStream_t stream);
hipError_t launch_gae(const NmmoExperience& x, const int32_t* idxs, int B, float g, float gl, float* adv,
                      hipStream_t stream);
hipError_t launch_gather_rows(const void* src, int64_t row_words, const int32_t* idx, int n, void* out,
                              hipStream_t stream);
hipError_t launch_policy(const PolicyParams& p, hipStream_t stream);
hipError_t launch_wrap(const WrapParams& p, int mode, hipStream_t stream);

}
```

### nmmo_amd/csrc/tick.hip

```cpp
#include "agent_obs.h"
#include "kernels.h"

namespace nmmo {

struct Ctx {
  int16_t* T;
  int16_t* ent_g;
  uint64_t* vism;
  int* gstart;
  uint32_t* glist;
  int16_t* rslot;
  uint32_t* pp;
  int* hkey;
  int* hmin;
  int16_t* amove;
  int16_t* atgt;
  int16_t* asty;
  int* ft;
  int16_t* clist;
  int16_t* ring;
  uint32_t* dep;
  int* E;
  int* wtot;
  int wsel;
// ... 1806 lines not shown
      int* mr = mi + (round & 1) * S;
      if (active) {
        atomicMax(&mr[s], key);
        atomicMax(&mr[t], key);
        anyf[round % 3] = 1;
      }
      if (tid == 0) anyf[(round + 1) % 3] = 0;
      __syncthreads();
      if (!anyf[round % 3]) break;
      if (active && mr[s] == key && mr[t] == key) {
        const int dmg = eval_attack(c, s, sty, t, eq_off, sys(c, NMMO_SYS_EQUIPMENT) ? c.clist[t] : 0);
        if (dmg >= 0) apply_attack(c, s, sty, t, dmg, tick);
        active = false;
      }
    }
  }
  NMMO_STAMP(25);
  if (evon && combat) {
    const int dm = s < P ? c.ev_dmg[s] : -1, lv = s < P ? c.ev_lvl[s] : 0, kv = s < P ? c.kill[s] : -1;
    ev_append(c, evn, (dm >= 0) + (lv > 0) + (kv >= 0), [&](int i) {
      const int sk = c.asty[s] + 1;
      if (dm >= 0) ev_put(c, i++, s, EV_SCORE_HIT, sk, 0, dm, 0, 0);
      if (lv > 0) ev_put(c, i++, s, EV_LEVEL_UP, sk, lv, 0, 0, 0);
      if (kv >= 0) {
        const int vl = max((int)TF(F_MELEE_LEVEL, kv), max((int)TF(F_RANGE_LEVEL, kv), (int)TF(F_MAGE_LEVEL, kv)));
        ev_put(c, i++, s, EV_PLAYER_KILL, 0, vl, 0, 0, TF(F_ID, kv));
      }
    });
  }
  NMMO_STAMP(26);
  if (items || sys(c, NMMO_SYS_EXCHANGE)) {
    uint32_t* victim = reinterpret_cast<uint32_t*>(c.misc);
    if (tid < 16) victim[tid] = 0u;
    __syncthreads();
    if (s < P && c.kill[s] >= 0) atomicOr(&victim[c.kill[s] >> 5], 1u << (c.kill[s] & 31));
    __syncthreads();
    int16_t* shot_row = c.clist;
    int freed = -1;
    const bool is_victim = s < S && ((victim[s >> 5] >> (s & 31)) & 1u);
    if (s < P && c.fired[s] && !is_victim) {
      freed = fire_ammo_deferred(c, s, c.asty[s]);
      c.fired[s] = 0;
    }
    if (s < P) shot_row[s] = (int16_t)freed;
    const bool nd = s < P && (c.fired[s] || c.kill[s] >= 0 || freed >= 0);
    int nn;
    const int pos = block_prefix_count(nd, wtot_next(c), &nn);
    if (nd) c.order[pos] = (int16_t)s;
    __syncthreads();
    NMMO_STAMP(27);
    if (tid == 0) {
      for (int i = 0; i < nn; i++) {
        const int x = c.order[i];
        if (shot_row[x] >= 0) ifree(c, shot_row[x]);
        if (c.fired[x]) fire_ammo(c, x, c.asty[x]);
        if (c.kill[x] >= 0) loot(c, x, c.kill[x], evn);
      }
      c.E[E_EVENT_COUNT] = evn;
    }
    __syncthreads();
    evn = c.E[E_EVENT_COUNT];
  }
  NMMO_STAMP(5);

  int gf = 0;
  if (inslot && c.amove[s] >= 0 && TF(F_ALIVE, s) && TF(F_HEALTH, s) > 0) {
    const int d = c.amove[s];
    const int nr = TF(F_ROW, s) + dir_dr(d), nc = TF(F_COL, s) + dir_dc(d);
    if ((d == 4 || ((nbm >> d) & 1u)) && TF(F_FREEZE, s) <= 0) {
      TF(F_ROW, s) = (int16_t)nr;
      TF(F_COL, s) = (int16_t)nc;
      const int progress = 64 - linf(80, 80, nr, nc);
      if (progress > TF(F_EXPLORATION, s)) {
        TF(F_EXPLORATION, s) = (int16_t)progress;
        gf = s < P ? progress : 0;
      }
    }
  }
  uint2 sw = make_uint2(0u, 0u);
  if (c.exch && s < P && sell_row >= 0 && acts(c, s)) {
    uint2* inv = c.inv + s * kInv;
    const int k = inv_find(inv, sell_row);
    if (k >= 0 && !it_equipped(inv[k])) {
      inv[k].x = (inv[k].x & 0x3FFu) | ((uint32_t)sell_price << 10) | ((uint32_t)tick << 17);
      sw = inv[k];
    }
  }
  if (evon) {
    const int nl = it_type(sw) ? 1 : 0;
    int tot;
    const int pre = block_prefix_sum((gf > 0 ? 1 : 0) | (nl << 16), wtot_next(c), &tot);
    c.ev_end = evn + (tot & 0xFFFF) + (tot >> 16);
    if (gf > 0) ev_put(c, evn + (pre & 0xFFFF), s, EV_GO_FARTHEST, 0, 0, gf, 0, 0);
    if (nl)
      ev_put(c, evn + (tot & 0xFFFF) + (pre >> 16), s, EV_LIST_ITEM, it_type(sw), it_level(sw), it_qty(sw),
             sell_price, 0);
    evn += (tot & 0xFFFF) + (tot >> 16);
  }
  NMMO_STAMP(6);

  const bool dead = inslot && TF(F_ALIVE, s) && TF(F_HEALTH, s) <= 0;
  const int ring_tail = c.E[E_FREE_HEAD] + c.E[E_FREE_COUNT];
  const int iring_tail = items ? c.E[E_ITEM_FREE_HEAD] + c.E[E_ITEM_FREE_COUNT] : 0;
  uint2* dinv = items ? c.inv + (s < P ? s : 0) * kInv : nullptr;
  const int nitem = (items && dead && s < P) ? inv_count(dinv) : 0;
  static_assert(kMaxSlots < 1024 && kInv * 128 < (1 << 14), "cull scan fields");
  int ctot;
  const int cpre = block_prefix_sum((dead ? 1 : 0) | ((dead && s < P) ? 1 << 10 : 0) | nitem << 18, wtot_next(c), &ctot);
  const int dpos = cpre & 1023, ppos = (cpre >> 10) & 255;
  const int ndead = ctot & 1023, npdead = (ctot >> 10) & 255;
  if (s < P) c.died[s] = dead ? 1 : 0;
  if (evon) {
    c.ev_end = evn + npdead;
    if (dead && s < P) ev_put(c, evn + ppos, s, EV_AGENT_CULLED, 0, 0, 0, 0, 0);
    evn += npdead;
  }
  if (dead) {
    c.ring[(ring_tail + dpos) % S] = TF(F_DS_ROW, s);
    TF(F_ALIVE, s) = 0;
    if (s < P) TF(F_DIED_TICK, s) = (int16_t)(tick + 1);
  }
  if (nitem) {
    const int base = iring_tail + (cpre >> 18);
    for (int k = 0; k < nitem; k++) {
      c.iring[(base + k) % c.IC] = (int16_t)it_row(dinv[k]);
      dinv[k] = make_uint2(0u, 0u);
    }
    TF(F_ITEM_LEVEL, s) = 0;
  }
  if (tid == 0) {
    c.E[E_FREE_COUNT] += ndead;
    c.E[E_PLAYERS_ALIVE] -= npdead;
    if (items) c.E[E_ITEM_FREE_COUNT] += ctot >> 18;
  }
  if (sys(c, NMMO_SYS_NPC) && ndead > npdead) {
    const bool keep = s >= P && inslot && TF(F_ALIVE, s);
    int nkeep;
    const int kpos = block_prefix_count(keep, wtot_next(c), &nkeep);
    int16_t v[kNFLive];
    if (keep) {
#pragma unroll
      for (int row = 0; row < kNFLive; row++)
        if (row < c.nf) v[row] = c.T[row * S + s];
    }
    __syncthreads();
    if (keep) {
#pragma unroll
      for (int row = 0; row < kNFLive; row++)
        if (row < c.nf) c.T[row * S + P + kpos] = v[row];
    }
    if (s >= P + nkeep && inslot) {
#pragma unroll
      for (int row = 0; row < kNFLive; row++)
        if (row < c.nf) c.T[row * S + s] = 0;
    }
    if (tid == 0) c.E[E_NPC_COUNT] = nkeep;
  }
  __syncthreads();
  NMMO_STAMP(7);

  const int rskip = !sys(c, NMMO_SYS_NPC) && (nt >> 6) >= 4 && P <= 128 ? 2 : 0;
  if ((tid >> 6) >= rskip) {
    const uint8_t* base = c.bank + (size_t)c.E[E_MAP_ID] * kTiles;
    const uint32_t* base4 = reinterpret_cast<const uint32_t*>(base);
    const bool foilage_only = !c.prof && !c.foreign;
    const int lane = lane_id(), wv = (tid >> 6) - rskip, nwv = (nt >> 6) - rskip;
    const int wcap = (128 * NW * 4) / nwv;
    int16_t* wlist = reinterpret_cast<int16_t*>(c.vism) + wv * wcap;
    const uint32_t rtick = (uint32_t)(tick + 1);
    auto groups_of = [&](int w) {
      uint32_t nz = w < kBitmapWords ? c.dep[w] : 0u;
      nz |= nz >> 1;
      nz |= nz >> 2;
      return nz & 0x11111111u;
    };
    int ng = 0;
    for (int ch = wv * 64; ch < kBitmapWords; ch += nwv * 64) {
      const int w = ch + lane;
      uint32_t nz = groups_of(w);
      const int n = __popc(nz);
      const int inc = wave_incl_scan(n);
      int k = ng + inc - n;
      ng += __builtin_amdgcn_readlane(inc, 63);
      while (nz) {
        const int b = __builtin_ctz(nz);
        nz &= nz - 1;
        if (k < wcap) wlist[k] = (int16_t)(w * 8 + (b >> 2));
        k++;
      }
    }
    NMMO_STAMP(16);
    if (ng <= wcap) {
      __builtin_amdgcn_fence(__ATOMIC_RELEASE, "wavefront");
      __builtin_amdgcn_wave_barrier();
      __builtin_amdgcn_fence(__ATOMIC_ACQUIRE, "wavefront");
      NMMO_STAMP(18);
      constexpr int kB = 4;
      for (int i0 = lane; i0 < ng; i0 += kB * 64) {
        int gb[kB];
        uint32_t b4[kB];
#pragma unroll
        for (int q = 0; q < kB; q++) {
          gb[q] = wlist[min(i0 + 64 * q, ng - 1)];
          b4[q] = foilage_only ? (uint32_t)M_FOILAGE * 0x01010101u : base4[gb[q]];
        }
#pragma unroll
        for (int q = 0; q < kB; q++) {
          if (i0 + 64 * q >= ng) break;
          const int g = gb[q], w = g >> 3, sh = (g & 7) * 4;
          const uint32_t nib = (c.dep[w] >> sh) & 15u;
          const U4 u = draw(seed, rtick, P_RESPAWN, (uint32_t)g, 0);
          const uint32_t uu[4] = {u.x, u.y, u.z, u.w};
          uint32_t clear = 0;
#pragma unroll
          for (int j = 0; j < 4; j++) {
            const int bm = (int)((b4[q] >> (8 * j)) & 255u);
            if (((nib >> j) & 1u) && uu[j] < respawn_u32(bm)) {
              c.mat[4 * g + j] = (uint8_t)bm;
              clear |= 1u << (sh + j);
            }
          }
          if (clear) atomicAnd(&c.dep[w], ~clear);
        }
      }
    } else {
      for (int ch = wv * 64; ch < kBitmapWords; ch += nwv * 64) {
        const int w = ch + lane;
        if (w >= kBitmapWords) continue;
        uint32_t bits = c.dep[w], keepb = bits;
        while (bits) {
          const int b = __builtin_ctz(bits);
          bits &= bits - 1;
          const int tt = w * 32 + b;
          const int bm = foilage_only ? (int)M_FOILAGE : base[tt];
          const U4 u = draw(seed, rtick, P_RESPAWN, (uint32_t)(tt >> 2), 0);
          const uint32_t ut = (tt & 3) == 0 ? u.x : (tt & 3) == 1 ? u.y : (tt & 3) == 2 ? u.z : u.w;
          if (ut < respawn_u32(bm)) {
            c.mat[tt] = (uint8_t)bm;
            keepb &= ~(1u << b);
          }
        }
        c.dep[w] = keepb;
      }
    }
  }
  if (!task_early) {
    tsr = c.tsg[s < P ? s : 0];
    tk = c.tasks[my_task];
  }
  if (c.exch && s < P) {
    uint2* inv = c.inv + s * kInv;
    for (int k = 0; k < kInv; k++) {
      if (!it_type(inv[k])) break;
      if (it_price(inv[k]) && tick + 1 - it_ltick(inv[k]) > 5) inv[k].x &= 0x3FFu;
    }
  }
  NMMO_STAMP(19);
  if (sys(c, NMMO_SYS_NPC) ? c.foreign_any : c.tmap) __syncthreads();
  if (tid == 0) c.E[E_TICK] = tick + 1;
  NMMO_STAMP(8);
  if (sys(c, NMMO_SYS_NPC)) npc_spawn(c, (uint32_t)(tick + 1), spawn, spawn_drawn);
  NMMO_STAMP(9);

  const int alive_n = c.E[E_PLAYERS_ALIVE];
  const bool done = alive_n == 0 || tick + 1 >= c.cfg->horizon || alive_n <= c.cfg->early_stop_agent_num;
  if (tid == 0) {
    c.E[E_DONE] = done;
    if (c.evcap) c.E[E_EVENT_COUNT] = evn;
  }
  if (c.tsee) {
    uint32_t* sw = reinterpret_cast<uint32_t*>(c.ft);
    for (int k = tid; k < ((c.S + 3) & ~3); k += blockDim.x)
      sw[k] = k < c.S && TF(F_ALIVE, k) ? (uint32_t)(TF(F_DS_ROW, k) & 511) << 16 | (uint32_t)(TF(F_ROW, k) & 255) << 8 |
                                              (uint32_t)(TF(F_COL, k) & 255)
                                        : 511u << 16;
    __syncthreads();
  }
  if (s < P) {
    float rw = 0.f;
    launder(tk);
    if (!c.tev) launder(tsr);
    if (c.pres[s] && c.died[s]) {
      rw = -1.f;
    } else if (c.pres[s]) {
      NmmoTaskState ts = c.tev ? c.tsl[s] : tsr;
      const double np = task_progress(c, s, tk, ts.acc), d = np - ts.last;
      ts.last = np;
      if (np > ts.max_progress) ts.max_progress = np;
      if (d > 0.0) ts.signals += 1;
      if (np >= 1.0 && ts.completed_tick == 0) ts.completed_tick = tick + 1;
      if (c.tev)
        c.tsl[s] = ts;
      else
        c.tsg[s] = ts;
      rw = (float)d;
    }
    rew[s] = rw;
    term[s] = c.died[s];
    trunc[s] = (uint8_t)(done && TF(F_ALIVE, s));
    mask[s] = c.pres[s];
  }
}

template <int kS, int kP>
__device__ __forceinline__ void wire_count_fused(Ctx& c, const DevState& st, int e) {
  static_assert(kS > 0 && kS <= kMaxSlots && kP > 0 && kP <= 128, "a specialised shape");
  auto al16 = [](size_t x) { return (x + 15) & ~(size_t)15; };
  constexpr size_t kIdBytes = (size_t)kIdWords * 4 * 2;
  constexpr size_t kRegion = union_lds_bytes(kS, true) + al16((size_t)(kS + 1) * 2) + 128 * 4 + 4 * al16((size_t)kS * 2) +
                             (size_t)kBitmapWords * 4 + NMMO_NE * 4 + 32 * 4 + 16 * 4 + 128 + 128;
  static_assert(kRegion >= kIdBytes, "the id set fits the union .. died range");
  constexpr size_t kSmall = (size_t)kMaxSlots * 8 + kMaxSlots / 8 + 128 + 16 * 4 + 4;
  static_assert(kSmall <= al16((size_t)kInv * kP * 2) + al16((size_t)(kInv * kP + 1) * 2), "the item ring and row map");
  constexpr uint32_t kOut = 0xFFFFFFFFu;
  const int tid = threadIdx.x, lane = lane_id(), S = kS, P = kP;
  const int w = __builtin_amdgcn_readfirstlane(wave_id()), nw = blockDim.x >> 6;
  int nm = 0;
  if (c.exch && tid == 0) {
    for (int j = 0; j < kLWords; j++) nm += __popcll(c.lbits[j]);
    nm = min(nm, NMMO_MARKET_ROWS);
  }
  const int s = tid;
  const bool in = s < S && TF(F_ALIVE, s);
  const int ds = s < S ? TF(F_DS_ROW, s) : 0, r = s < S ? TF(F_ROW, s) : 0, col = s < S ? TF(F_COL, s) : 0;
  const int id = s < S ? TF(F_ID, s) : 0, ta = s < S ? TF(F_TIME_ALIVE, s) : 0, npc = s < S ? TF(F_NPC_TYPE, s) : 0;
  int ninv = 0;
  if (tid < P) {
    const uint2* inv = c.inv + tid * kInv;
#pragma unroll
    for (int k = kInv - 1; k >= 0; k--) ninv = it_type(inv[k]) ? ninv + 1 : 0;
  }
  __syncthreads();
  uint32_t* pk = reinterpret_cast<uint32_t*>(c.iring);
  uint32_t* pos = pk + kMaxSlots;
  uint32_t* tab = pos + kMaxSlots;
  uint8_t* nin = reinterpret_cast<uint8_t*>(tab + kMaxSlots / 32);
  int* wsum = reinterpret_cast<int*>(nin + 128);
  int* bytes = wsum + 16;
  uint32_t* ids = reinterpret_cast<uint32_t*>(c.vism);
  int* pre = reinterpret_cast<int*>(ids + kIdWords);
  for (int k = tid; k < kMaxSlots; k += blockDim.x) pk[k] = kOut;
  if (tid < kMaxSlots / 32) tab[tid] = 0u;
  idset_clear(ids);
  if (tid < P) nin[tid] = (uint8_t)ninv;
  if (tid == 0) *bytes = 0;
  __syncthreads();
  if (s < kMaxSlots) {
    pos[s] = in ? ((uint32_t)(uint16_t)r << 16) | (uint32_t)(uint16_t)col : kOut;
    if (in && (unsigned)(ds - 1) < (unsigned)S) {
      const bool player = s < P;
      pk[ds - 1] = ao_pack(s, r, col, player && ta < st.wf.spawn_immunity, npc > 1, player);
    }
  }
  __syncthreads();
  const WireView v = wire_view(st.wf.wire, st.wf.n_envs, P);
  uint32_t pr[kMaxSlots / 64];
#pragma unroll
  for (int i = 0; i < kMaxSlots / 64; i++) {
    pr[i] = pk[lane + 64 * i];
    if (w == 0) st.wf.wpk[(size_t)e * kMaxSlots + lane + 64 * i] = pr[i];
  }
  int mine = 0;
  for (int a = w; a < P; a += nw) {
    const uint32_t pa = pos[a];
    uint32_t word = 0u;
    if (pa != kOut) {
      const uint32_t rc = (pa >> 16) | (pa & 0xFFFFu) << 16;
      int nvis = 0;
#pragma unroll
      for (int i = 0; i < kMaxSlots / 64; i++) {
        const uint32_t x = pr[i];
        const bool iw = ao_in_window(x, rc);
        const uint64_t b = __ballot(iw);
        if (iw && nvis + __popcll(b & lanes_below()) < kNObs) {
          const int q = ao_slot(x);
          atomicOr(&tab[q >> 5], 1u << (q & 31));
        }
        nvis += __popcll(b);
      }
      word = wire_count_word(min(nvis, kNObs), nin[a]);
    }
    if (lane == 0) {
      v.cnt[(size_t)e * P + a] = (uint16_t)word;
      mine += wire_record_bytes(word);
    }
  }
  if (lane == 0) atomicAdd(bytes, mine);
  __syncthreads();
  const bool shown = s < S && ((tab[s >> 5] >> (s & 31)) & 1u);
  if (shown) idset_add(ids, id);
  const int ne = idset_prefix(ids, pre, wsum);
  if (s < kMaxSlots) st.wf.wrank[(size_t)e * kMaxSlots + s] = shown ? (uint16_t)idrank(ids, pre, id) : (uint16_t)0xFFFF;
  if (tid == 0) {
    v.mcount[e] = (uint16_t)nm;
    v.ecount[e] = (uint16_t)ne;
    v.env_off[e] = wire_table_bytes(ne) + *bytes + 32 * nm;
  }
}

__device__ __forceinline__ void store_market(Ctx& c, const DevState& st, int e) {
  const int tid = threadIdx.x;
  if (!c.exch) {
    if (tid == 0) st.mcount[e] = 0;
    return;
  }
  build_market(c);
  int32_t* ml = st.mlist + (size_t)e * NMMO_MARKET_ROWS;
  for (int row = tid + 1; row <= c.IC; row += blockDim.x) {
    const int w = row >> 6;
    const uint64_t m = c.lbits[w];
    if (!((m >> (row & 63)) & 1)) continue;
    int rank = __popcll(m & ((1ull << (row & 63)) - 1ull));
    for (int j = 0; j < w; j++) rank += __popcll(c.lbits[j]);
    if (rank < NMMO_MARKET_ROWS) {
      const int rm = c.rmap[row];
      ml[rank] = row | ((rm & 255) << 16) | ((rm >> 8) << 24);
    }
  }
  if (tid == 0) {
    int n = 0;
    for (int j = 0; j < kLWords; j++) n += __popcll(c.lbits[j]);
    st.mcount[e] = min(n, NMMO_MARKET_ROWS);
  }
}

template <uint32_t kSys, int kS, int kP>
__device__ __forceinline__ void tick_body(const DevState& st, const int32_t* __restrict__ actions,
                                          const uint64_t* __restrict__ env_seeds, float* rew, uint8_t* term,
                                          uint8_t* trunc, uint8_t* mask, int mode) {
  extern __shared__ __attribute__((aligned(16))) unsigned char smem[];
  const int e = st.env_list ? st.env_list[blockIdx.x] : (int)blockIdx.x;
  if ((unsigned)e >= (unsigned)st.n_envs) {
    if (threadIdx.x == 0) atomicCAS(st.fault, 0, NMMO_FAULT_ENV_LIST | (int)blockIdx.x << 8);
    return;
  }
  NMMO_STAMP_CLEAR();
  NMMO_STAMP(0);
  Ctx c = make_ctx<kS, kP>(smem, st, e, kSys ? kSys : st.cfg.systems);
  Heads hd = {};
  if (mode == 0) {
    const int32_t* a = actions + ((size_t)e * c.P + min((int)threadIdx.x, c.P - 1)) * kHeads;
#pragma unroll
    for (int k = 0; k < kHeads; k++)
      if (k == 0 || k == 1 || k == 8 || c.items) hd.v[k] = a[k];
  }
  const bool defer = defer_dep(c, kSys);
  const DepQ dq = load_env(c, st, e, kSys == NMMO_SYS_RESOURCE, defer);
  __syncthreads();
  NMMO_STAMP(20);
  const size_t o = (size_t)e * c.P;
  const bool reset_path = mode == 1 || c.E[E_DONE];
  const int alive0 = c.E[E_PLAYERS_ALIVE];
  const int ev_start = c.E[E_EVENT_COUNT];
  if (reset_path) {
    const int env_global = (int)(st.cfg.env_index_base + (uint64_t)e);
    uint64_t seed;
    int episode;
    if (mode == 1) {
      seed = env_seeds ? env_seeds[e] : splitmix64(st.seed ^ splitmix64((uint64_t)env_global));
      episode = 0;
    } else {
      seed = splitmix64(env_seed(c) ^ (0xD1B54A32D192ED03ull * (uint64_t)(c.E[E_EPISODE] + 1)));
      episode = c.E[E_EPISODE] + 1;
    }
    __syncthreads();
    reset_env(c, seed, episode, env_global);
    for (int i = threadIdx.x; i < c.P * (int)sizeof(NmmoTaskState) / 4; i += blockDim.x) {
      if (c.tev)
        reinterpret_cast<int*>(c.tsl)[i] = 0;
      else
        reinterpret_cast<int*>(c.tsg)[i] = 0;
    }
    if (!c.items) {
      for (int i = threadIdx.x; i < c.P * kInv; i += blockDim.x) st.items[(size_t)e * c.P * kInv + i] = make_uint2(0u, 0u);
      for (int i = threadIdx.x; i < c.IC; i += blockDim.x) st.iring[(size_t)e * c.IC + i] = (int16_t)(i + 1);
    }
    for (int p = threadIdx.x; p < c.P; p += blockDim.x) {
      if (rew) rew[o + p] = 0.f;
      if (term) term[o + p] = 0;
      if (trunc) trunc[o + p] = 0;
      if (mask) mask[o + p] = 1;
    }
  } else {
    tick_env(c, hd, defer, dq, rew + o, term + o, trunc + o, mask + o);
  }
  __syncthreads();
  if (st.counters && threadIdx.x == 0) {
    const bool reset = mode == 1 || reset_path;
    atomicAdd(&st.counters[0], (unsigned long long)(reset ? c.P : alive0));
    if (!reset && c.E[E_DONE]) atomicAdd(&st.counters[1], 1ull);
    if (!reset && c.evcap) atomicAdd(&st.counters[2], (unsigned long long)(c.E[E_EVENT_COUNT] - ev_start));
  }
  NMMO_STAMP(10);
  store_market(c, st, e);
  store_env(c, st, e);
  if constexpr (kSys == NMMO_SYS_ALL && kS > 0 && kP > 0)
    if (st.wf.wire) wire_count_fused<kS, kP>(c, st, e);
#ifdef NMMO_STAMPS
  __syncthreads();
#endif
  NMMO_STAMP(11);
}

template <uint32_t kSys, int kS = 0, int kP = 0>
__global__ void tick_kernel(DevState st, const int32_t* __restrict__ actions,
                            const uint64_t* __restrict__ env_seeds, float* rew, uint8_t* term,
                            uint8_t* trunc, uint8_t* mask, int mode) {
  tick_body<kSys, kS, kP>(st, actions, env_seeds, rew, term, trunc, mask, mode);
}
#ifndef NMMO_TICK_C3_WPE
#define NMMO_TICK_C3_WPE 8
#endif
template <uint32_t kSys, int kS = 0, int kP = 0>
__global__ void __attribute__((amdgpu_waves_per_eu(NMMO_TICK_C3_WPE, NMMO_TICK_C3_WPE)))
tick_kernel_w8(DevState st, const int32_t* __restrict__ actions, const uint64_t* __restrict__ env_seeds,
               float* rew, uint8_t* term, uint8_t* trunc, uint8_t* mask, int mode) {
  tick_body<kSys, kS, kP>(st, actions, env_seeds, rew, term, trunc, mask, mode);
}


hipError_t launch_tick(const DevState& st, const int32_t* actions, const uint64_t* env_seeds,
                       float* rew, uint8_t* term, uint8_t* trunc, uint8_t* mask, int mode,
                       hipStream_t stream) {
#ifndef NMMO_TICK_MIN_THREADS
#define NMMO_TICK_MIN_THREADS 512
#endif
  const int threads = max(((st.S + 63) / 64) * 64, NMMO_TICK_MIN_THREADS);
  const size_t lds = tick_lds_bytes(st.S, st.P, (st.cfg.systems & NMMO_SYS_ITEM) != 0, st.tev != 0,
                                    uses_grid(st.cfg.systems), slim_systems(st.cfg.systems));
  void (*k)(DevState, const int32_t*, const uint64_t*, float*, uint8_t*, uint8_t*, uint8_t*, int);
  const bool s128 = st.S == 128 && st.P == 128, s384 = st.S == 384 && st.P == 128;
  switch (st.cfg.systems) {
    case kSysC2: k = s128 ? tick_kernel<kSysC2, 128, 128> : tick_kernel<kSysC2>; break;
    case kSysC3: k = s384 ? tick_kernel_w8<kSysC3, 384, 128> : tick_kernel_w8<kSysC3>; break;
    case NMMO_SYS_ALL: k = s384 ? tick_kernel<NMMO_SYS_ALL, 384, 128> : tick_kernel<NMMO_SYS_ALL>; break;
    default: k = tick_kernel<0>; break;
  }
  const int grid = list_grid(st.env_list, st.n_list, st.n_envs);
  if (grid <= 0) return hipSuccess;
  hipLaunchKernelGGL(k, dim3(grid), dim3(threads), lds, stream,
                     st, actions, env_seeds, rew, term, trunc, mask, mode);
  return hipGetLastError();
}

hipError_t init_kernels() {
  const void* ks[7] = {reinterpret_cast<const void*>(tick_kernel<kSysC2>),
                       reinterpret_cast<const void*>(tick_kernel_w8<kSysC3>),
                       reinterpret_cast<const void*>(tick_kernel<NMMO_SYS_ALL>),
                       reinterpret_cast<const void*>(tick_kernel<0>),
                       reinterpret_cast<const void*>(tick_kernel<kSysC2, 128, 128>),
                       reinterpret_cast<const void*>(tick_kernel_w8<kSysC3, 384, 128>),
                       reinterpret_cast<const void*>(tick_kernel<NMMO_SYS_ALL, 384, 128>)};
  for (const void* k : ks) {
    hipFuncAttributes fa;
    hipError_t err = hipFuncGetAttributes(&fa, k);
    if (err != hipSuccess) return err;
    err = hipFuncSetAttribute(k, hipFuncAttributeMaxDynamicSharedMemorySize, (int)(160 * 1024 - fa.sharedSizeBytes));
    if (err != hipSuccess) return err;
  }
  return hipSuccess;
}

__global__ void rebuild_dep_kernel(DevState st) {
  __shared__ uint64_t lbits[kLWords];
  __shared__ int16_t rmap[kInv * 128 + 1];
  const int e = blockIdx.x, tid = threadIdx.x;
  const int32_t* E = st.env + (size_t)e * NMMO_NE;
  const uint8_t* mat = st.mat + (size_t)e * kTiles;
  const uint8_t* base = st.bank + (size_t)E[E_MAP_ID] * kTiles;
  bool foreign = false;
  for (int w = tid; w < kBitmapWords; w += blockDim.x) {
    uint32_t bits = 0;
    for (int b = 0; b < 32; b++) {
      const bool d = mat[w * 32 + b] != base[w * 32 + b];
      bits |= (d ? 1u : 0u) << b;
      foreign = foreign || (d && base[w * 32 + b] != M_FOILAGE);
    }
    st.dep[(size_t)e * kBitmapWords + w] = bits;
  }
  if (__ballot(foreign) && lane_id() == 0) atomicOr(st.foreign, 1);
  if (tid < kLWords) lbits[tid] = 0;
  __syncthreads();
  const bool exch = (st.cfg.systems & NMMO_SYS_ITEM) && (st.cfg.systems & NMMO_SYS_EXCHANGE);
  if (exch && tid < st.P) {
    const uint2* inv = st.items + ((size_t)e * st.P + tid) * kInv;
    for (int k = 0; k < kInv && it_type(inv[k]); k++)
      if (it_price(inv[k])) {
        const int row = it_row(inv[k]);
        rmap[row] = (int16_t)(tid | (k << 8));
        atomicOr((unsigned long long*)&lbits[row >> 6], 1ull << (row & 63));
      }
  }
  __syncthreads();
  if (tid == 0) {
    int n = 0;
    for (int row = 1; row <= kInv * st.P; row++)
      if ((lbits[row >> 6] >> (row & 63)) & 1) {
        if (n < NMMO_MARKET_ROWS)
          st.mlist[(size_t)e * NMMO_MARKET_ROWS + n] = row | ((rmap[row] & 255) << 16) | ((rmap[row] >> 8) << 24);
        n++;
      }
    st.mcount[e] = min(n, NMMO_MARKET_ROWS);
  }
}

hipError_t launch_rebuild_dep(const DevState& st, hipStream_t stream) {
  const hipError_t err = hipMemsetAsync(st.foreign, 0, 4, stream);
  if (err != hipSuccess) return err;
  hipLaunchKernelGGL(rebuild_dep_kernel, dim3(st.n_envs), dim3(256), 0, stream, st);
  return hipGetLastError();
}

}

#ifdef NMMO_STAMPS
extern "C" __attribute__((visibility("default"))) int nmmo_debug_read_stamps(unsigned long long* out,
                                                                              int n) {
  return (int)hipMemcpyFromSymbol(out, HIP_SYMBOL(nmmo::g_stamps), (size_t)n * 8, 0,
                                  hipMemcpyDeviceToHost);
}
#endif
```

Measured before the change: 341.5 million.

## Fuse flat-obs entity mirror and packed slots into tick kernel epilogue

At the end of the tick kernel, each env now writes a row-major mirror of per-slot entity columns (32 int16 per slot) plus the packed visibility words into new global buffers. A specialised flat_obs kernel variant reads these instead of restaging the column-major entity table into LDS. It gathers the first 12 visible entity rows per agent up front with vector loads and computes the visibility compaction for all of a wave's agents before the window stage. This is meant to cut LDS staging and shrink the obs kernel's shared-memory footprint, at the cost of extra global writes in tick and extra allocations. It applies only to the flat layout, all systems, S=384 and P=128, and only when the zero-row tag is active.

```diff
diff --git a/nmmo_amd/csrc/agent_obs.h b/nmmo_amd/csrc/agent_obs.h
--- a/nmmo_amd/csrc/agent_obs.h
+++ b/nmmo_amd/csrc/agent_obs.h
@@ -174,16 +174,17 @@
 struct AoNoop {
   __device__ void operator()() const {}
 };
-template <int kAgents = kAoAgents, int kRowDw = kAoWinRowBytes / 4, typename F = AoNoop, typename B = AoNoop>
-__device__ inline void ao_stage_windows(const ObsParams& p, int e, int g, const int16_t* T, int Sp, uint32_t* ws, uint2* is,
-                                        F before_barrier = F(), B before_writes = B()) {
+template <int kAgents = kAoAgents, int kRowDw = kAoWinRowBytes / 4, bool kAlways = false, typename F = AoNoop,
+          typename B = AoNoop>
+__device__ __forceinline__ void ao_stage_windows_at(const ObsParams& p, int e, int g, int pr, int pc, uint32_t* ws, uint2* is,
+                                           F before_barrier = F(), B before_writes = B()) {
   static_assert(kRowDw == 4 || kRowDw == 5, "window row: 5 aligned dwords, or 4 realigned");
   const int tid = threadIdx.x, P = p.P;
   const int la = tid / 15, row = tid - 15 * la, a = g * kAgents + la;
   const bool win = tid < kAgents * 15 && a < P;
   uint32_t d[5] = {0u, 0u, 0u, 0u, 0u};
-  if (win) {
-    const int r = ao_clamp_pos(T[F_ROW * Sp + a]), c = ao_clamp_pos(T[F_COL * Sp + a]);
+  if (kAlways || win) {
+    const int r = ao_clamp_pos(pr), c = ao_clamp_pos(pc);
     const int base = (r - kVision + row) * kSize + c - kVision;
     const uint32_t* src = reinterpret_cast<const uint32_t*>(p.mat + (size_t)e * kTiles) + (base >> 2);
 #pragma unroll
@@ -195,15 +196,24 @@
   }
   uint2 iw = make_uint2(0u, 0u);
   const bool itm = tid < kAgents * kInv && g * kAgents + tid / kInv < P;
-  if (itm) iw = p.items[((size_t)e * P + g * kAgents) * kInv + tid];
+  if constexpr (kAlways) iw = p.items[(size_t)e * P * kInv + min(g * kAgents * kInv + tid, P * kInv - 1)];
+  else if (itm) iw = p.items[((size_t)e * P + g * kAgents) * kInv + tid];
   before_writes();
   if (win) {
 #pragma unroll
     for (int k = 0; k < kRowDw; k++) ws[tid * kRowDw + k] = d[k];
   }
-  if (tid < kAgents * kInv) is[tid] = iw;
+  if (tid < kAgents * kInv) is[tid] = kAlways && !itm ? make_uint2(0u, 0u) : iw;
   before_barrier();
   __syncthreads();
+}
+template <int kAgents = kAoAgents, int kRowDw = kAoWinRowBytes / 4, typename F = AoNoop, typename B = AoNoop>
+__device__ inline void ao_stage_windows(const ObsParams& p, int e, int g, const int16_t* T, int Sp, uint32_t* ws, uint2* is,
+                                        F before_barrier = F(), B before_writes = B()) {
+  const int tid = threadIdx.x, a = g * kAgents + tid / 15;
+  const bool win = tid < kAgents * 15 && a < p.P;
+  ao_stage_windows_at<kAgents, kRowDw, false>(p, e, g, win ? T[F_ROW * Sp + a] : 0, win ? T[F_COL * Sp + a] : 0, ws, is,
+                                       before_barrier, before_writes);
 }
 template <int kRowBytes = kAoWinRowBytes>
 __device__ __forceinline__ void ao_win_offsets(int (&wo)[2]) {
diff --git a/nmmo_amd/csrc/capi.hip b/nmmo_amd/csrc/capi.hip
--- a/nmmo_amd/csrc/capi.hip
+++ b/nmmo_amd/csrc/capi.hip
@@ -49,6 +49,8 @@
   uint64_t* d_zext = nullptr;
   bool zskip = true;
   bool wire_fuse = true;
+  int16_t* d_frows = nullptr;
+  bool flat_fuse = true;
   const void* zbuf = nullptr;
   uint64_t ztag = 0;
   unsigned long long* d_rows_out = nullptr;
@@ -167,7 +169,8 @@
   void* bufs[] = {h->d_env,  h->d_ent,   h->d_ring,  h->d_mat,   h->d_dep,   h->d_bank,
                   h->d_task, h->d_seeds, h->d_items, h->d_iring, h->d_mlist, h->d_mcount,
                   h->d_events, h->d_tasks, h->d_assign, h->d_tstate, h->d_ws, h->d_uniq, h->d_wenv, h->d_wdrop, h->d_task_cum,
-                  h->d_wcount, h->d_wmcount, h->d_wrank, h->d_wpk, h->d_foreign, h->d_zrow, h->d_zext};
+                  h->d_wcount, h->d_wmcount, h->d_wrank, h->d_wpk, h->d_foreign, h->d_zrow, h->d_zext,
+                  h->d_frows};
   for (void* b : bufs)
     if (b) (void)hipFree(b);
   delete h;
@@ -233,6 +236,12 @@
     h->zskip = !(rz && rz[0] == '1');
     const char* wf = getenv("NMMO_WIRE_FUSE");
     h->wire_fuse = !(wf && wf[0] == '0');
+    const char* ff = getenv("NMMO_FLAT_FUSE");
+    h->flat_fuse = !(ff && ff[0] == '0');
+  }
+  if (cfg->obs_layout == NMMO_OBS_FLAT && h->flat_fuse && cfg->systems == NMMO_SYS_ALL && S == 384 && P == 128) {
+    ALLOC(h->d_wpk, n * (size_t)kMaxSlots * 4);
+    ALLOC(h->d_frows, n * (size_t)S * kMirrorCols * 2);
   }
   if (cfg->obs_layout == NMMO_OBS_WIRE) {
     ALLOC(h->d_wrank, n * (size_t)kMaxSlots * 2);
@@ -290,6 +299,8 @@
   p.zext = h->d_zext;
   p.ztag = h->d_zrow && h->zskip && obs && obs == h->zbuf ? h->ztag : 0;
   p.rows_out = h->d_rows_out;
+  p.fpk = nullptr;
+  p.frows = nullptr;
   p.counted = 0;
   p.recs = nullptr;
   p.fault_dst = nullptr;
@@ -373,6 +384,13 @@
     st.wf.n_envs = st.n_envs;
     st.wf.spawn_immunity = h->cfg.spawn_immunity;
   }
+  const bool mirror = do_obs && h->d_frows && h->cfg.obs_layout == NMMO_OBS_FLAT && obs_params(h, obs).ztag != 0 &&
+                      st.cfg.systems == NMMO_SYS_ALL && st.S == 384 && st.P == 128;
+  if (mirror) {
+    st.fm.pk = h->d_wpk;
+    st.fm.rows = h->d_frows;
+    st.fm.spawn_immunity = h->cfg.spawn_immunity;
+  }
   if (rec) HIP_TRY(hipEventRecord(ev[0], s));
   HIP_TRY(launch_tick(st, actions, nullptr, rew, term, trunc, mask, 0, s));
   if (rec) HIP_TRY(hipEventRecord(ev[1], s));
@@ -388,6 +406,10 @@
     op.env_list = env_ids;
     op.n_list = n_ids;
     op.counted = st.wf.wire != nullptr;
+    if (mirror) {
+      op.fpk = h->d_wpk;
+      op.frows = h->d_frows;
+    }
     if (op.wire && h->d_recs) {
       op.recs = h->d_recs;
       op.fault_dst = h->d_recs_fault;
diff --git a/nmmo_amd/csrc/flat_obs.hip b/nmmo_amd/csrc/flat_obs.hip
--- a/nmmo_amd/csrc/flat_obs.hip
+++ b/nmmo_amd/csrc/flat_obs.hip
@@ -54,6 +54,15 @@
                   (5 * fo_lds_bytes(kMaxSlots) <= 160 * 1024 && fo_items_in_T(kMaxSlots) &&
                    5 * ((fo_lds_bytes(kMaxSlots) + kFoLdsGranule - 1) / kFoLdsGranule * kFoLdsGranule) <= 160 * 1024),
               "5 workgroups per CU");
+
+constexpr int kFoGather = 12;
+static_assert(kFoGather % 4 == 0 && kFoGather <= 16 && kFoGather <= kNObs, "gathered rows");
+constexpr size_t kFoOwnBytes = (size_t)kAoAgents * kMirrorCols * 2;
+constexpr size_t kFoGatBytes = (size_t)kAoAgents * kFoGather * kMirrorCols * 2;
+constexpr size_t kFoMirrorLds =
+    kFoOwnBytes + kFoGatBytes + (size_t)kFoListPool + (size_t)kAoAgents * kFoVisw * 4 + kFoWinBytes + kFoItemBytes;
+static_assert(5 * ((kFoMirrorLds + kFoLdsGranule - 1) / kFoLdsGranule * kFoLdsGranule) <= 160 * 1024 &&
+                  kFoOwnBytes % 16 == 0 && kFoGatBytes % 16 == 0, "5 workgroups per CU");
 
 template <int kSh>
 __device__ __forceinline__ uint64_t fo_shift(uint64_t lo, uint64_t hi) {
@@ -191,18 +200,22 @@
 
 typedef const __attribute__((address_space(4))) ObsParams* FoArgs;
 
-template <bool kWrap, int kS, bool kAligned = true>
+template <bool kWrap, int kS, bool kAligned = true, bool kMirror = false>
 __global__ void __launch_bounds__(64 * kAoWaves) __attribute__((amdgpu_waves_per_eu(5, 5))) flat_obs_kernel(ObsParams p) {
+  static_assert(!kMirror || (kS == kMaxSlots && kAligned), "the mirror variant: 384 slots");
   extern __shared__ __attribute__((aligned(16))) unsigned char smem[];
   const int S = kS ? kS : p.S, P = p.P, Sp = ao_stride(S), tdim = p.task_dim, elems = kFlatTask + tdim + kTileN;
+  constexpr int kPerWave = kAoAgents / kAoWaves;
+  static_assert(!kMirror || (kPerWave * kFoGather) % 16 == 0, "gather: 16 rows per load instruction");
   int16_t* T = reinterpret_cast<int16_t*>(smem);
-  uint16_t* mpo = reinterpret_cast<uint16_t*>(smem + ao_columns_lds(S));
+  int16_t* gat = reinterpret_cast<int16_t*>(smem + kFoOwnBytes);
+  uint16_t* mpo = reinterpret_cast<uint16_t*>(smem + (kMirror ? kFoOwnBytes + kFoGatBytes : ao_columns_lds(S)));
   uint32_t* visw_all = reinterpret_cast<uint32_t*>(mpo) + kFoListPool / 4;
   uint2* mtop = reinterpret_cast<uint2*>(visw_all) - 1;
-  uint32_t* wst = visw_all + kAoWaves * kFoVisw;
+  uint32_t* wst = visw_all + (kMirror ? kAoAgents : kAoWaves) * kFoVisw;
   uint32_t* pk = wst;
-  uint2* ist = reinterpret_cast<uint2*>(fo_items_in_T(S) ? smem + (size_t)F_ROW * Sp * 2
-                                                         : reinterpret_cast<unsigned char*>(wst) + kFoWinBytes);
+  uint2* ist = reinterpret_cast<uint2*>(!kMirror && fo_items_in_T(S) ? smem + (size_t)F_ROW * Sp * 2
+                                                                     : reinterpret_cast<unsigned char*>(wst) + kFoWinBytes);
 #if NMMO_FO_XCD
   int el, g;
   ao_env_group(p.env_list ? p.n_list : p.n_envs, (p.P + kAoAgents - 1) / kAoAgents, el, g);
@@ -218,9 +231,23 @@
 #endif
   const int w = __builtin_amdgcn_readfirstlane(wave_id());
   AoStage sg;
-  ao_stage_load<kAligned>(p, e, sg);
+  const int16_t* M = kMirror ? p.frows + (size_t)e * S * kMirrorCols : nullptr;
+  uint32_t pr[kAoRows];
+  uint4 ow = make_uint4(0u, 0u, 0u, 0u);
+  int wpr = 0, wpc = 0;
+  if constexpr (kMirror) {
+    sg.nm = p.mcount[e];
+    sg.mv = p.mlist[(size_t)e * NMMO_MARKET_ROWS + min(tid, NMMO_MARKET_ROWS - 1)];
+#pragma unroll
+    for (int i = 0; i < kAoRows; i++) pr[i] = p.fpk[(size_t)e * kMaxSlots + lane + 64 * i];
+    ow = reinterpret_cast<const uint4*>(M + (size_t)min(g * kAoAgents + ((tid >> 2) & (kAoAgents - 1)), P - 1) * kMirrorCols)[tid & 3];
+    const int16_t* wr = M + (size_t)min(g * kAoAgents + tid / 15, P - 1) * kMirrorCols;
+    wpr = wr[F_ROW];
+    wpc = wr[F_COL];
+  } else {
+    ao_stage_load<kAligned>(p, e, sg);
+  }
   const int16_t* E = p.ent + (size_t)e * NMMO_NF * S;
-  constexpr int kPerWave = kAoAgents / kAoWaves;
   const int abase = g * kAoAgents + w;
   int my_task = 0, my_prev = -1, my_alive = 0;
   uint64_t my_z = 0, my_s = 0;
@@ -229,7 +256,7 @@
     const int aj = min(abase + kAoWaves * min(lane, kPerWave - 1), P - 1);
     const size_t ai = (size_t)e * P + aj;
     my_task = p.assign[ai];
-    my_alive = E[F_ALIVE * S + aj];
+    my_alive = kMirror ? M[(size_t)aj * kMirrorCols + kMirrorCols - 1] : E[F_ALIVE * S + aj];
     if (p.zrow) {
       my_z = p.zrow[ai];
       my_s = p.zst[ai];
@@ -237,13 +264,19 @@
     if constexpr (kWrap)
       if (p.ws) my_prev = p.ws[ai].prev_price;
   }
-  ao_stage_store<kAligned>(p, e, T, pk, sg);
+  uint32_t my_rc;
+  if constexpr (kMirror) {
+    const int16_t* mr = M + (size_t)min(abase + kAoWaves * min(lane, kPerWave - 1), P - 1) * kMirrorCols;
+    my_rc = (uint32_t)(uint16_t)mr[F_ROW] | (uint32_t)(uint16_t)mr[F_COL] << 16;
+    if (tid < kAoAgents * 4) reinterpret_cast<uint4*>(T)[tid] = ow;
+  } else {
+    ao_stage_store<kAligned>(p, e, T, pk, sg);
+  }
   if (!mine) {
     my_task = 0, my_prev = -1, my_alive = 0;
     my_z = my_s = 0;
   }
-  uint32_t my_rc;
-  {
+  if constexpr (!kMirror) {
     const int aj = min(abase + kAoWaves * min(lane, kPerWave - 1), P - 1);
     my_rc = (uint32_t)(uint16_t)T[F_ROW * Sp + aj] | (uint32_t)(uint16_t)T[F_COL * Sp + aj] << 16;
   }
@@ -251,10 +284,40 @@
   wst_[1] = __builtin_amdgcn_s_memtime();
 #endif
 
-  uint32_t pr[kAoRows];
-#pragma unroll
-  for (int i = 0; i < kAoRows; i++) pr[i] = pk[lane + 64 * i];
-  uint32_t* visw = visw_all + w * kFoVisw;
+  if constexpr (!kMirror) {
+#pragma unroll
+    for (int i = 0; i < kAoRows; i++) pr[i] = pk[lane + 64 * i];
+  }
+  uint32_t* visw = visw_all + w * (kMirror ? kPerWave : 1) * kFoVisw;
+  int my_nv = 0;
+  constexpr int kGatIt = kPerWave * kFoGather / 16;
+  static_assert(kGatIt >= 1 && kGatIt <= 4, "gather loads");
+  uint4 gq0, gq1, gq2, gq3;
+  gq0 = gq1 = gq2 = gq3 = make_uint4(0u, 0u, 0u, 0u);
+  if constexpr (kMirror) {
+#pragma unroll
+    for (int j = 0; j < kPerWave; j++) {
+      int nvj = 0;
+      if (__builtin_amdgcn_readlane(my_alive, j) && !(NMMO_FO_ABL & 32)) {
+        const int rcj = __builtin_amdgcn_readlane((int)my_rc, j);
+        nvj = min(fo_compact(pr, (int16_t)(rcj & 0xFFFF), rcj >> 16, visw + j * kFoVisw), kNObs);
+      }
+      if (lane == j) my_nv = nvj;
+    }
+    __builtin_amdgcn_fence(__ATOMIC_RELEASE, "wavefront");
+    __builtin_amdgcn_wave_barrier();
+    __builtin_amdgcn_fence(__ATOMIC_ACQUIRE, "wavefront");
+    auto gather = [&](int i) {
+      const int t = (lane >> 2) + 16 * i, tj = t / kFoGather, tk = t - tj * kFoGather;
+      const uint32_t vw = visw[tj * kFoVisw + tk];
+      const int slot = tk < __shfl(my_nv, tj) ? ao_slot(vw) : 0;
+      return reinterpret_cast<const uint4*>(M + (size_t)min(slot, S - 1) * kMirrorCols)[lane & 3];
+    };
+    gq0 = gather(0);
+    if constexpr (kGatIt > 1) gq1 = gather(1);
+    if constexpr (kGatIt > 2) gq2 = gather(2);
+    if constexpr (kGatIt > 3) gq3 = gather(3);
+  }
   const uint8_t* wsb = reinterpret_cast<const uint8_t*>(wst);
   const float tickf = (float)p.env[(size_t)e * NMMO_NE + E_TICK];
   const bool exch = (p.systems & NMMO_SYS_ITEM) && (p.systems & NMMO_SYS_EXCHANGE);
@@ -268,7 +331,7 @@
   const int ja = lane < 40 ? lane / 10 : lane - 40, ji = lane / 12;
   const bool img_ok = lane < 44 && abase + kAoWaves * ja < P && ((zextv >> ja) & 1);
   const bool pinv_ok = lane < 48 && abase + kAoWaves * ji < P && ((zextv >> ji) & 1);
-  if (p.zext) {
+  if (kMirror || p.zext) {
     const int aa = min(abase + kAoWaves * min(ja, kPerWave - 1), P - 1);
     const int ai = min(abase + kAoWaves * min(ji, kPerWave - 1), P - 1);
     img = reinterpret_cast<const uint2*>(p.zext)[((size_t)e * P + aa) * kZext + (lane < 40 ? lane % 10 : 10)];
@@ -276,7 +339,14 @@
   }
   const int nm = min(max(sg.nm, 0), NMMO_MARKET_ROWS), nst = fo_staged(nm);
   const uint2 lwd = ao_listing_load(p, e, sg);
-  ao_stage_windows<kAoAgents, kFoWinRowBytes / 4>(p, e, g, T, Sp, wst, ist, [&]() {
+  auto listings = [&]() {
+    if constexpr (kMirror) {
+      uint4* gd = reinterpret_cast<uint4*>(gat) + w * kGatIt * 64 + lane;
+      gd[0] = gq0;
+      if constexpr (kGatIt > 1) gd[64] = gq1;
+      if constexpr (kGatIt > 2) gd[128] = gq2;
+      if constexpr (kGatIt > 3) gd[192] = gq3;
+    }
     if (tid < nm) {
       mpo[tid] = (uint16_t)(it_price(lwd) | ((sg.mv >> 16) & 255) << 8);
       if (tid < nst) mtop[-tid] = lwd;
@@ -288,7 +358,11 @@
       mpo[j] = (uint16_t)(it_price(wd) | own << 8);
       if (j < nst) mtop[-j] = wd;
     }
-  }, []() { __syncthreads(); });
+  };
+  if constexpr (kMirror)
+    ao_stage_windows_at<kAoAgents, kFoWinRowBytes / 4, true>(p, e, g, wpr, wpc, wst, ist, listings);
+  else
+    ao_stage_windows<kAoAgents, kFoWinRowBytes / 4>(p, e, g, T, Sp, wst, ist, listings, []() { __syncthreads(); });
 #if NMMO_FO_STAMPS
   wst_[2] = __builtin_amdgcn_s_memtime();
 #endif
@@ -361,8 +435,11 @@
     const int la = a - g * kAoAgents;
     const int rcj = __builtin_amdgcn_readlane((int)my_rc, j);
     const int r = (int16_t)(rcj & 0xFFFF), c = rcj >> 16;
-    const int gold = __builtin_amdgcn_readfirstlane(T[F_GOLD * Sp + a]);
-    const int aid = __builtin_amdgcn_readfirstlane(T[F_ID * Sp + a]);
+    const int16_t* Ta = kMirror ? T + la * kMirrorCols : T;
+    const int Spa = kMirror ? 1 : Sp, tia = kMirror ? 0 : a;
+    if constexpr (kMirror) visw = visw_all + (w * kPerWave + j) * kFoVisw;
+    const int gold = __builtin_amdgcn_readfirstlane(Ta[F_GOLD * Spa + tia]);
+    const int aid = __builtin_amdgcn_readfirstlane(Ta[F_ID * Spa + tia]);
     const uint8_t* wa = wsb + la * kFoWinAgentBytes;
     uint32_t wm[4];
 #pragma unroll
@@ -370,10 +447,15 @@
     const uint2 it = lane < kInv ? ist[la * kInv + lane] : make_uint2(0u, 0u);
     const uint32_t mv = ao_move_bits(wm[1]);
     const int ninv = __builtin_ctzll(~__ballot(lane < kInv && it_type(it) != 0));
-    const int nv = (NMMO_FO_ABL & 32) ? 0 : min(fo_compact(pr, r, c, visw), kNObs);
-    __builtin_amdgcn_fence(__ATOMIC_RELEASE, "wavefront");
-    __builtin_amdgcn_wave_barrier();
-    __builtin_amdgcn_fence(__ATOMIC_ACQUIRE, "wavefront");
+    int nv;
+    if constexpr (kMirror) {
+      nv = __builtin_amdgcn_readlane(my_nv, j);
+    } else {
+      nv = (NMMO_FO_ABL & 32) ? 0 : min(fo_compact(pr, r, c, visw), kNObs);
+      __builtin_amdgcn_fence(__ATOMIC_RELEASE, "wavefront");
+      __builtin_amdgcn_wave_barrier();
+      __builtin_amdgcn_fence(__ATOMIC_ACQUIRE, "wavefront");
+    }
 
     FO_STAMP(1);
     const bool ext = (zextv >> j) & 1;
@@ -381,7 +463,7 @@
     if (!(NMMO_FO_ABL & 1)) {
       AoAgent ag;
       ag.a = a;
-      ag.ti = a;
+      ag.ti = tia;
       ag.r = r;
       ag.c = c;
       ag.gold = gold;
@@ -390,7 +472,7 @@
       ag.ninv = ninv;
       ag.prev_price = kWrap ? __builtin_amdgcn_readlane(my_prev, j) : -1;
       ag.mv = mv;
-      const AoSections x = ao_sections<kWrap>(p, T, Sp, visw, ag, it);
+      const AoSections x = ao_sections<kWrap>(p, Ta, Spa, visw, ag, it);
       FO_STAMP(2);
       fg.ext = ext;
       fo_put<0>(row, fg, fo_chunk<0>(x), 0.f, 0.f);
@@ -425,17 +507,37 @@
       const uint32_t de = kFlatEntity + (lane - eh);
       const bool epos = (lane & 31) == F_ROW || (lane & 31) == F_COL;
       const uint32_t esh = (lane & 31) == F_COL ? 16u : 0u;
+      const int16_t* gj = gat + (size_t)(w * kPerWave + j) * kFoGather * kMirrorCols;
+      const int nst2 = kMirror ? min(nv2, kFoGather) : nv2;
 #pragma unroll 1
-      for (int k0 = 0; k0 < nv2; k0 += 2) {
+      for (int k0 = 0; k0 < nst2; k0 += 2) {
         const int k = k0 + eh;
         if (ef < NMMO_N_ENTITY_COLS) {
           float v = 0.f;
           if (k < nv) {
             const uint32_t vw = visw[k];
-            const int tv = T[ef * Sp + ao_slot(vw)];
+            const int tv = kMirror ? gj[k * kMirrorCols + ef] : T[ef * Sp + ao_slot(vw)];
             v = (float)(epos ? (int)((vw >> esh) & 255u) : tv);
           }
           fo_st(row, de + k0 * NMMO_N_ENTITY_COLS, v);
+        }
+      }
+      if constexpr (kMirror) {
+        if (nv2 > kFoGather) {
+          const int16_t* Mk = kp->frows + (size_t)e * kMaxSlots * kMirrorCols;
+#pragma unroll 1
+          for (int k0 = kFoGather; k0 < nv2; k0 += 2) {
+            const int k = k0 + eh;
+            if (ef < NMMO_N_ENTITY_COLS) {
+              float v = 0.f;
+              if (k < nv) {
+                const uint32_t vw = visw[k];
+                const int tv = Mk[(size_t)min(ao_slot(vw), kMaxSlots - 1) * kMirrorCols + ef];
+                v = (float)(epos ? (int)((vw >> esh) & 255u) : tv);
+              }
+              fo_st(row, de + k0 * NMMO_N_ENTITY_COLS, v);
+            }
+          }
         }
       }
       const int hz = max(nv2, hv);
@@ -524,9 +626,11 @@
     if (lane == 0 && (size_t)e * P + a < (1u << 17))
       for (int k = 0; k < kFoStamps; k++) fo_stamp_buf[(size_t)e * P + a][k] = fst[k];
 #endif
-    __builtin_amdgcn_fence(__ATOMIC_RELEASE, "wavefront");
-    __builtin_amdgcn_wave_barrier();
-    __builtin_amdgcn_fence(__ATOMIC_ACQUIRE, "wavefront");
+    if constexpr (!kMirror) {
+      __builtin_amdgcn_fence(__ATOMIC_RELEASE, "wavefront");
+      __builtin_amdgcn_wave_barrier();
+      __builtin_amdgcn_fence(__ATOMIC_ACQUIRE, "wavefront");
+    }
   }
 #if NMMO_FO_STAMPS
   wst_[4] = __builtin_amdgcn_s_memtime();
@@ -553,7 +657,11 @@
   const dim3 grid(ne, (p.P + kAoAgents - 1) / kAoAgents), block(64 * kAoWaves);
 #endif
   const size_t lds = fo_lds_bytes(p.S);
-  if (p.S == kMaxSlots) {
+  if (p.frows) {
+    if (!p.fpk || !p.zext || p.S != kMaxSlots) return hipErrorInvalidValue;
+    if (p.wflags) hipLaunchKernelGGL((flat_obs_kernel<true, kMaxSlots, true, true>), grid, block, kFoMirrorLds, stream, p);
+    else hipLaunchKernelGGL((flat_obs_kernel<false, kMaxSlots, true, true>), grid, block, kFoMirrorLds, stream, p);
+  } else if (p.S == kMaxSlots) {
     if (p.wflags) hipLaunchKernelGGL((flat_obs_kernel<true, kMaxSlots>), grid, block, lds, stream, p);
     else hipLaunchKernelGGL((flat_obs_kernel<false, kMaxSlots>), grid, block, lds, stream, p);
   } else if (p.S % 8 != 0) {
diff --git a/nmmo_amd/csrc/kernels.h b/nmmo_amd/csrc/kernels.h
--- a/nmmo_amd/csrc/kernels.h
+++ b/nmmo_amd/csrc/kernels.h
@@ -51,7 +51,14 @@
     int n_envs;
     int spawn_immunity;
   } wf;
-};
+  struct FlatMirror {
+    uint32_t* pk;
+    int16_t* rows;
+    int spawn_immunity;
+  } fm;
+};
+constexpr int kMirrorCols = 32;
+static_assert(NMMO_N_ENTITY_COLS < kMirrorCols, "mirror row");
 __host__ __device__ inline int list_grid(const int32_t* list, int n_list, int n) { return list ? n_list : n; }
 
 struct ObsParams {
@@ -90,6 +97,8 @@
   const uint8_t* trunc;
   const uint8_t* mask;
   unsigned long long* rows_out;
+  const uint32_t* fpk;
+  const int16_t* frows;
 };
 constexpr uint64_t kZsZero = 1ull << 20;
 constexpr uint64_t kZsExt = 1ull << 21;
diff --git a/nmmo_amd/csrc/tick.hip b/nmmo_amd/csrc/tick.hip
--- a/nmmo_amd/csrc/tick.hip
+++ b/nmmo_amd/csrc/tick.hip
@@ -2132,6 +2132,26 @@
   }
 }
 
+struct SlotPack {
+  bool in;
+  int ds, r, col, id, ta, npc;
+};
+template <int kS>
+__device__ __forceinline__ SlotPack slot_pack_read(const Ctx& c, int s) {
+  SlotPack v;
+  v.in = s < kS && TF(F_ALIVE, s);
+  v.ds = s < kS ? TF(F_DS_ROW, s) : 0, v.r = s < kS ? TF(F_ROW, s) : 0, v.col = s < kS ? TF(F_COL, s) : 0;
+  v.id = s < kS ? TF(F_ID, s) : 0, v.ta = s < kS ? TF(F_TIME_ALIVE, s) : 0, v.npc = s < kS ? TF(F_NPC_TYPE, s) : 0;
+  return v;
+}
+template <int kS, int kP>
+__device__ __forceinline__ void slot_pack_put(uint32_t* pk, int s, const SlotPack& v, int spawn_immunity) {
+  if (s < kMaxSlots && v.in && (unsigned)(v.ds - 1) < (unsigned)kS) {
+    const bool player = s < kP;
+    pk[v.ds - 1] = ao_pack(s, v.r, v.col, player && v.ta < spawn_immunity, v.npc > 1, player);
+  }
+}
+
 template <int kS, int kP>
 __device__ __forceinline__ void wire_count_fused(Ctx& c, const DevState& st, int e) {
   static_assert(kS > 0 && kS <= kMaxSlots && kP > 0 && kP <= 128, "a specialised shape");
@@ -2151,9 +2171,9 @@
     nm = min(nm, NMMO_MARKET_ROWS);
   }
   const int s = tid;
-  const bool in = s < S && TF(F_ALIVE, s);
-  const int ds = s < S ? TF(F_DS_ROW, s) : 0, r = s < S ? TF(F_ROW, s) : 0, col = s < S ? TF(F_COL, s) : 0;
-  const int id = s < S ? TF(F_ID, s) : 0, ta = s < S ? TF(F_TIME_ALIVE, s) : 0, npc = s < S ? TF(F_NPC_TYPE, s) : 0;
+  const SlotPack sv = slot_pack_read<kS>(c, s);
+  const bool in = sv.in;
+  const int r = sv.r, col = sv.col, id = sv.id;
   int ninv = 0;
   if (tid < P) {
     const uint2* inv = c.inv + tid * kInv;
@@ -2177,10 +2197,7 @@
   __syncthreads();
   if (s < kMaxSlots) {
     pos[s] = in ? ((uint32_t)(uint16_t)r << 16) | (uint32_t)(uint16_t)col : kOut;
-    if (in && (unsigned)(ds - 1) < (unsigned)S) {
-      const bool player = s < P;
-      pk[ds - 1] = ao_pack(s, r, col, player && ta < st.wf.spawn_immunity, npc > 1, player);
-    }
+    slot_pack_put<kS, kP>(pk, s, sv, st.wf.spawn_immunity);
   }
   __syncthreads();
   const WireView v = wire_view(st.wf.wire, st.wf.n_envs, P);
@@ -2226,6 +2243,37 @@
     v.ecount[e] = (uint16_t)ne;
     v.env_off[e] = wire_table_bytes(ne) + *bytes + 32 * nm;
   }
+}
+
+template <int kS, int kP>
+__device__ __forceinline__ void flat_mirror_fused(Ctx& c, const DevState& st, int e) {
+  static_assert(kS > 0 && kS <= kMaxSlots && kS % 64 == 0 && kP > 0 && kP <= 128, "a specialised shape");
+  static_assert((size_t)kMaxSlots * 4 <= (((size_t)kInv * kP * 2 + 15) & ~(size_t)15), "the item ring");
+  static_assert(NMMO_N_ENTITY_COLS == 31 && kMirrorCols == 32, "mirror row");
+  const int tid = threadIdx.x, s = tid;
+  const SlotPack sv = slot_pack_read<kS>(c, s);
+  if (s < kS) {
+    uint4* dst = reinterpret_cast<uint4*>(st.fm.rows + ((size_t)e * kS + s) * kMirrorCols);
+#pragma unroll
+    for (int q = 0; q < 4; q++) {
+      uint32_t d[4];
+#pragma unroll
+      for (int k = 0; k < 4; k++) {
+        const int f = 8 * q + 2 * k;
+        const uint32_t lo = (uint16_t)TF(f, s);
+        const uint32_t hi = f + 1 < NMMO_N_ENTITY_COLS ? (uint16_t)TF(f + 1, s) : (uint16_t)TF(F_ALIVE, s);
+        d[k] = lo | hi << 16;
+      }
+      dst[q] = make_uint4(d[0], d[1], d[2], d[3]);
+    }
+  }
+  __syncthreads();
+  uint32_t* pk = reinterpret_cast<uint32_t*>(c.iring);
+  for (int k = tid; k < kMaxSlots; k += blockDim.x) pk[k] = kAoEmpty;
+  __syncthreads();
+  slot_pack_put<kS, kP>(pk, s, sv, st.fm.spawn_immunity);
+  __syncthreads();
+  for (int k = tid; k < kMaxSlots; k += blockDim.x) st.fm.pk[(size_t)e * kMaxSlots + k] = pk[k];
 }
 
 __device__ __forceinline__ void store_market(Ctx& c, const DevState& st, int e) {
@@ -2324,8 +2372,10 @@
   NMMO_STAMP(10);
   store_market(c, st, e);
   store_env(c, st, e);
-  if constexpr (kSys == NMMO_SYS_ALL && kS > 0 && kP > 0)
+  if constexpr (kSys == NMMO_SYS_ALL && kS > 0 && kP > 0) {
     if (st.wf.wire) wire_count_fused<kS, kP>(c, st, e);
+    else if (st.fm.rows) flat_mirror_fused<kS, kP>(c, st, e);
+  }
 #ifdef NMMO_STAMPS
   __syncthreads();
 #endif
```

Result: faster. 353.0 million, median of 6 (+3.4%).
